# crowsonkb/k-diffusion

Measured on AMD Instinct MI355X. Metric: images/sec, 256x256 image_transformer_v2, 50-step DPM++2M (whole job), higher is better.
Workload: dtype f32

## Files before the change

### k-diffusion_amd/csrc/attn_ffn_x3.hip

```cpp
#include "attn_x3_core.h"
#include "ffn_x3h_core.h"

namespace kd {
namespace x3 {

extern unsigned long long* g_clk;

constexpr int AF_KS = 7;
constexpr int AF_LDS_FFN = 4 * STG + 4 * 1024 + 4 * 2048;
constexpr int AF_LDS = x3a::NaGeo<AF_KS>::LDS > AF_LDS_FFN ? x3a::NaGeo<AF_KS>::LDS : AF_LDS_FFN;
static_assert(AF_LDS <= 80 * 1024, "two workgroups per CU");

struct PanelTile {
  static constexpr bool ATT_LDS = true;
  int tok0, W;
  __device__ __forceinline__ int row(int i) const { return tok0 + (4 * (i >> 6) + ((i & 31) >> 3)) * W + 8 * ((i >> 5) & 1) + (i & 7); }
};

__global__ __launch_bounds__(256, 2) void attn_ffn_x3h_kernel(const x3a::NArgs a, const FArgs3 p) {
  using namespace x3a;
  extern __shared__ __attribute__((aligned(16))) char smem[];
  const int tid = threadIdx.x;
  const auto warm = code_warm_begin<28 * 1024>((int)blockIdx.x < a.warm && tid < 64);
  (void)wg_stamp_begin(a.clk);
  const int tiles_x = a.W / NA_TW, tiles_y = a.H / NA_TH;
  int r = KD_XCD_CHUNK();
  const int tx = r % tiles_x; r /= tiles_x;
  const int ty = r % tiles_y, b = r / tiles_y;
  auto fresh = [&]() { int t = tid; asm volatile("" : "+v"(t)); return t; };

  f32x4 on[2][2][4];
  static_for<2>([&](auto head_) {
    constexpr int head = decltype(head_)::value;
    na2d_x3_tile<AF_KS>(smem, a, fresh(), b, head, ty, tx, [&]() { if constexpr (head == 0) code_warm_end(warm); },
                        [&](bool, int, float l, const f32x16 (&O)[2]) {
      const float inv = 1.0f / l;
#pragma unroll
      for (int e = 0; e < 2; ++e)
#pragma unroll
        for (int g = 0; g < 4; ++g) on[head][e][g] = f32x4(f32x4{O[e][4 * g], O[e][4 * g + 1], O[e][4 * g + 2], O[e][4 * g + 3]} * inv);
    });
    KD_BARRIER();
  });

  const int tid_b = fresh();
  {
    const int lane = tid_b & 63, wid = __builtin_amdgcn_readfirstlane(tid_b >> 6), l31 = lane & 31, h2 = lane >> 5;
    char* rowp = smem + wid * STG + l31 * 512;
#pragma unroll
    for (int head = 0; head < 2; ++head)
#pragma unroll
      for (int e = 0; e < 2; ++e)
#pragma unroll
        for (int g = 0; g < 4; ++g)
          *reinterpret_cast<f32x4*>(rowp + (((16 * head + 8 * e + 2 * g + h2) ^ (l31 & 15)) << 4)) = on[head][e][g];
  }
  asm volatile("s_waitcnt lgkmcnt(0)\n\t; kd_phase_b" ::: "memory");

  ffn_x3h_body<true>(p, smem, tid_b, PanelTile{(b * a.H + ty * NA_TH) * a.W + tx * NA_TW, a.W}, []() {});
  wg_stamp_end(wg_stamp_again(a.clk));
}

}
}

using namespace kd;

extern "C" int kd_attn_ffn_f32_supported(int batch, int H, int W, int nh, int ks, int K, int d_ff) {
  if (!opt(KD_OPT_attn_ffn_x3) || !opt(KD_OPT_attn_x3) || !opt(KD_OPT_ffn_x3)) return 0;
  if (ks != x3::AF_KS || nh != 2 || K != 128 || d_ff <= 0 || (d_ff & 63)) return 0;
  if (batch <= 0 || H <= 0 || W <= 0 || H % x3a::NA_TH || W % x3a::NA_TW) return 0;
  return kd_ffn_f32_supported(batch * H * W, K, d_ff);
}

extern "C" int kd_attn_ffn_f32(const float* qkv, const KdFfn* dp, int batch, int H, int W, int nh, int ks, void* stream) {
  if (!qkv || !dp) return fail(KD_EINVAL, "kd_attn_ffn_f32: null qkv / descriptor");
  const KdFfn& d = *dp;
  if (!d.x || !d.out || !d.scale || !d.Wp_up || !d.Wp_down || !d.Wp_out) return fail(KD_EINVAL, "kd_attn_ffn_f32: null x / out / scale / Wp_up / Wp_down / Wp_out");
  if (ks != x3::AF_KS || nh != 2 || d.K != 128 || d.d_ff <= 0 || (d.d_ff & 63) || batch <= 0 || H <= 0 || W <= 0 || H % x3a::NA_TH || W % x3a::NA_TW)
    return fail(KD_EINVAL, "kd_attn_ffn_f32: kernel size 7, 2 heads of 64, K = 128, d_ff a multiple of 64, token grid a multiple of 8 x 16 (ks=%d nh=%d K=%d d_ff=%d H=%d W=%d)",
                ks, nh, d.K, d.d_ff, H, W);
  if ((long long)batch * H * W != d.M || d.rows_per_sample != H * W || (d.scale_stride & 3))
    return fail(KD_EINVAL, "kd_attn_ffn_f32: M = batch H W, rows_per_sample = H W, scale_stride %% 4 == 0");
  x3a::NArgs a{qkv, nullptr, batch, H, W, nh, code_warm(), x3::g_clk};
  x3::FArgs3 f{};
  f.X = reinterpret_cast<const float*>(d.x); f.Y = reinterpret_cast<float*>(d.out);
  f.Wu = reinterpret_cast<const char*>(d.Wp_up); f.Wd = reinterpret_cast<const char*>(d.Wp_down);
  f.scale = d.scale; f.scale_stride = d.scale_stride; f.rows_per_sample = d.rows_per_sample; f.eps = d.eps;
  f.M = d.M; f.d_ff = d.d_ff; f.n_tiles = d.d_ff / 64;
  f.warm = 0;
  f.clk = x3::g_clk;
  f.Wo = reinterpret_cast<const char*>(d.Wp_out);
  const double M = d.M, K = d.K;
  const double flops = 4.0 * M * nh * x3a::DH * ks * ks + 2.0 * M * 3.0 * d.d_ff * K + 2.0 * M * K * K;
  const double bytes = 16.0 * M * nh * x3a::DH + 4.0 * (3.0 * M * K + 3.0 * d.d_ff * K + K * K) - 8.0 * M * K;
  const ProfName nm("attn_ffn_x3", "attn_ffn_x3 %dx%d nh=%d K=%d d_ff=%d", H, W, nh, d.K, d.d_ff);
  LaunchScope prof(nm, flops, bytes, (hipStream_t)stream);
  launch<x3::attn_ffn_x3h_kernel>(dim3((unsigned)(d.M / 128)), dim3(256), x3::AF_LDS, (hipStream_t)stream, a, f);
  return check_launch("kd_attn_ffn_f32");
}

KD_TEXT_PAD(attn_ffn_x3)
```

### k-diffusion_amd/csrc/attn_x3_core.h

```cpp
#pragma once
#include "x3_common.h"

namespace kd {
namespace x3a {


using b16::bf16x8;
using b16::u32x2;
using b16::u32x4;

constexpr int DH = 64;
constexpr int NA_TH = 8, NA_TW = 16;
constexpr int ROWB = 256;
template <int KS>
struct NaGeo {
  static constexpr int HR = NA_TH + KS - 1, HC = NA_TW + KS - 1;
  static constexpr int PR = 4 + KS - 1;
  static constexpr int NKT = (PR * 16 + 31) / 32;
  static constexpr int ROWS = ((HR * HC - KS + 9 + 3) / 4) * 4;
  static constexpr int LDS = ROWS * ROWB;
  static_assert(8 + KS - 1 <= 16, "16-key patch rows");
};

struct NArgs {
  const float* qkv; float* out;
  int batch, H, W, nh;
  int warm;
  unsigned long long* clk;
};

#define KD_WAIT_VM(n) asm volatile("s_waitcnt vmcnt(" #n ")" ::: "memory")

__device__ __forceinline__ void glds16(const void* src, void* dst) {
  __builtin_amdgcn_global_load_lds((const __attribute__((address_space(1))) void*)src, (__attribute__((address_space(3))) void*)dst, 16, 0, 0);
}

__device__ __forceinline__ int rsw(int row) { return ((row & 3) << 2) | ((row >> 2) & 3); }

using s16x4 = short __attribute__((ext_vector_type(4)));
__device__ __forceinline__ u32x2 tr_read(const char* img, int addr) {
  return __builtin_bit_cast(u32x2, __builtin_amdgcn_ds_read_tr16_b64_v4i16((s16x4 __attribute__((address_space(3)))*)(img + addr)));
}
__device__ __forceinline__ float max3f(float a, float b, float c) { return __builtin_fmaxf(__builtin_fmaxf(a, b), c); }
__device__ __forceinline__ float min3f(float a, float b, float c) { return __builtin_fminf(__builtin_fminf(a, b), c); }


template <int KS, class Mid, class Sink>
__device__ __forceinline__ void na2d_x3_tile(char* img, const NArgs& a, int tid, int b, int head, int ty, int tx, Mid&& mid, Sink&& sink) {
  using G = NaGeo<KS>;
  constexpr int HR = G::HR, HC = G::HC, PR = G::PR, NKT = G::NKT, ROWS = G::ROWS;
  const int lane = tid & 63, wid = __builtin_amdgcn_readfirstlane(tid >> 6), l31 = lane & 31, h2 = lane >> 5;
  const int wy_ = wid >> 1, wx_ = wid & 1;
  const int T = a.H * a.W;
  const size_t row_bytes = (size_t)3 * a.nh * DH * 4;
  const char* base = reinterpret_cast<const char*>(a.qkv) + (size_t)b * T * row_bytes + head * (DH * 4);
  const int ty0 = ty * NA_TH, tx0 = tx * NA_TW;
  const int hy0 = max(0, min(ty0 - KS / 2, a.H - HR)), hx0 = max(0, min(tx0 - KS / 2, a.W - HC));

  constexpr int NPC = (ROWS / 4 + 3) / 4;
  unsigned soff[NPC];
  {
    int row = 4 * wid + (lane >> 4);
    int y = row / HC, x = row % HC;
#pragma unroll
    for (int i = 0; i < NPC; ++i) {
      const int ky = min(hy0 + y, a.H - 1), kx = min(hx0 + x, a.W - 1);
      soff[i] = (unsigned)((ky * a.W + kx) * (int)row_bytes + (((lane & 15) ^ rsw(x)) << 4));
      x += 16;
      if (x >= HC) { x -= HC; ++y; }
    }
  }
  auto stage = [&](int part_bytes) {
#pragma unroll
    for (int i = 0; i < NPC; ++i) {
      const int pc = wid + 4 * i;
      if (pc < ROWS / 4) glds16(base + (size_t)soff[i] + part_bytes, img + pc * 1024);
    }
  };
  stage(a.nh * DH * 4);
  const int qy_raw = ty0 + 4 * wy_ + (l31 >> 3), qx_raw = tx0 + 8 * wx_ + (l31 & 7);
  const bool q_ok = qy_raw < a.H && qx_raw < a.W;
  const int qy = min(qy_raw, a.H - 1), qx = min(qx_raw, a.W - 1);
  const int q_tok = qy * a.W + qx;
  bf16x8 qa[4][2], ql[4];
  {
    const u32x4* qp = reinterpret_cast<const u32x4*>(base + (size_t)q_tok * row_bytes + 32 * h2);
#pragma unroll
    for (int st = 0; st < 4; ++st) {
      const u32x4 c0 = qp[4 * st], c1 = qp[4 * st + 1];
      qa[st][0] = __builtin_bit_cast(bf16x8, u32x4{c0[0], c0[1], c0[0], c0[1]});
      qa[st][1] = __builtin_bit_cast(bf16x8, u32x4{c1[0], c1[1], c1[0], c1[1]});
      ql[st] = __builtin_bit_cast(bf16x8, u32x4{c0[2], c0[3], c1[2], c1[3]});
    }
  }
  const int wy = max(0, min(qy - KS / 2, a.H - KS)) - hy0, wx = max(0, min(qx - KS / 2, a.W - KS)) - hx0;
  const int row_lo = min(max(0, min(min(ty0 + 4 * wy_, a.H - 1) - KS / 2, a.H - KS)) - hy0, HR - PR);
  const int col_lo = min(max(0, min(min(tx0 + 8 * wx_, a.W - 1) - KS / 2, a.W - KS)) - hx0, HC - (8 + KS - 1));
  const int korg = row_lo * HC + col_lo;
  float colv[8], rowv[2 * NKT];
  {
    const int r0 = wy - row_lo, c0 = wx - col_lo;
#pragma unroll
    for (int j = 0; j < 8; ++j) colv[j] = ((unsigned)((j & 3) + 8 * (j >> 2) + 4 * h2 - c0) < (unsigned)KS) ? INFINITY : -INFINITY;
#pragma unroll
    for (int p = 0; p < 2 * NKT; ++p) rowv[p] = ((unsigned)(p - r0) < (unsigned)KS) ? INFINITY : -INFINITY;
  }
  KD_WAIT_VM(0);
  mid();
  KD_BARRIER();

  f32x16 S[NKT];
#pragma unroll
  for (int t = 0; t < NKT; ++t)
#pragma unroll
    for (int i = 0; i < 16; ++i) S[t][i] = 0.f;
  const int kr0 = korg + (l31 >> 4) * HC + (l31 & 15);
  const int ka0 = kr0 * ROWB + (((2 * h2) ^ rsw(col_lo + (l31 & 15))) << 4);
#pragma unroll
  for (int st = 0; st < 4; ++st) {
    bf16x8 kc0[NKT], kc1[NKT], kh[NKT];
    const char* k0p = img + (ka0 ^ (st << 6));
    const char* k1p = img + (ka0 ^ (st << 6) ^ 16);
#pragma unroll
    for (int t = 0; t < NKT; ++t) {
      const u32x4 c0 = *reinterpret_cast<const u32x4*>(k0p + t * (2 * HC * ROWB));
      const u32x4 c1 = *reinterpret_cast<const u32x4*>(k1p + t * (2 * HC * ROWB));
      kc0[t] = __builtin_bit_cast(bf16x8, c0);
      kc1[t] = __builtin_bit_cast(bf16x8, c1);
      kh[t] = __builtin_bit_cast(bf16x8, u32x4{c0[0], c0[1], c1[0], c1[1]});
    }
#pragma unroll
    for (int t = 0; t < NKT; ++t) S[t] = __builtin_amdgcn_mfma_f32_32x32x16_bf16(kc0[t], qa[st][0], S[t], 0, 0, 0);
#pragma unroll
    for (int t = 0; t < NKT; ++t) S[t] = __builtin_amdgcn_mfma_f32_32x32x16_bf16(kc1[t], qa[st][1], S[t], 0, 0, 0);
#pragma unroll
    for (int t = 0; t < NKT; ++t) S[t] = __builtin_amdgcn_mfma_f32_32x32x16_bf16(kh[t], ql[st], S[t], 0, 0, 0);
  }
  asm volatile("s_waitcnt lgkmcnt(0)" ::: "memory");
  KD_BARRIER();
  stage(2 * a.nh * DH * 4);

#pragma unroll
  for (int t = 0; t < NKT; ++t)
#pragma unroll
    for (int i = 0; i < 16; ++i) S[t][i] = min3f(S[t][i], colv[i & 7], rowv[2 * t + (i >> 3)]);
  float m = -INFINITY;
#pragma unroll
  for (int t = 0; t < NKT; ++t)
#pragma unroll
    for (int i = 0; i < 16; i += 2) m = max3f(m, S[t][i], S[t][i + 1]);
  m = fmaxf(m, __shfl_xor(m, 32, 64));
  float l;
  {
    constexpr float LOG2E = 1.4426950408889634f;
    const f32x2 mb = {-m * LOG2E, -m * LOG2E};
    f32x2 l2 = {0.f, 0.f};
#pragma unroll
    for (int t = 0; t < NKT; ++t)
#pragma unroll
      for (int i = 0; i < 16; i += 2) {
        const f32x2 x = __builtin_elementwise_fma(f32x2{S[t][i], S[t][i + 1]}, f32x2{LOG2E, LOG2E}, mb);
        const f32x2 pv = {__builtin_amdgcn_exp2f(x.x), __builtin_amdgcn_exp2f(x.y)};
        S[t][i] = pv.x;
        S[t][i + 1] = pv.y;
        l2 += pv;
      }
    l = l2.x + l2.y;
  }
  l += __shfl_xor(l, 32, 64);
  bf16x8 ph[NKT][2], pl[NKT][2];
#pragma unroll
  for (int t = 0; t < NKT; ++t)
#pragma unroll
    for (int u = 0; u < 2; ++u) {
      u32x4 hi, lo;
      x3::split8(f32x4{S[t][8 * u], S[t][8 * u + 1], S[t][8 * u + 2], S[t][8 * u + 3]},
                 f32x4{S[t][8 * u + 4], S[t][8 * u + 5], S[t][8 * u + 6], S[t][8 * u + 7]}, hi, lo);
      ph[t][u] = __builtin_bit_cast(bf16x8, hi);
      pl[t][u] = __builtin_bit_cast(bf16x8, lo);
    }
  KD_WAIT_VM(0);
  KD_BARRIER();

  f32x16 O[2];
#pragma unroll
  for (int e = 0; e < 2; ++e)
#pragma unroll
    for (int i = 0; i < 16; ++i) O[e][i] = 0.f;
  const int vr0 = korg + 4 * h2 + ((lane & 15) >> 2);
  const int vc = (lane & 3) + 4 * ((lane >> 4) & 1);
  const int va0 = vr0 * ROWB + ((vc ^ rsw(col_lo + 4 * h2 + ((lane & 15) >> 2))) << 4);
  const int vb[2][2] = {{va0, (va0 ^ 32) + 8 * ROWB}, {va0 ^ 128, ((va0 ^ 128) ^ 32) + 8 * ROWB}};
#pragma unroll
  for (int t = 0; t < NKT; ++t)
#pragma unroll
    for (int u = 0; u < 2; ++u) {
      constexpr int step = HC * ROWB;
      bf16x8 vh[2], vl[2];
#pragma unroll
      for (int e = 0; e < 2; ++e) {
        const int a0 = vb[e][0] + (2 * t + u) * step, a1 = vb[e][1] + (2 * t + u) * step;
        const u32x2 h0 = tr_read(img, a0), h1 = tr_read(img, a1), l0 = tr_read(img, a0 + 8), l1 = tr_read(img, a1 + 8);
        vh[e] = __builtin_bit_cast(bf16x8, u32x4{h0[0], h0[1], h1[0], h1[1]});
        vl[e] = __builtin_bit_cast(bf16x8, u32x4{l0[0], l0[1], l1[0], l1[1]});
      }
      O[0] = __builtin_amdgcn_mfma_f32_32x32x16_bf16(vl[0], ph[t][u], O[0], 0, 0, 0);
      O[1] = __builtin_amdgcn_mfma_f32_32x32x16_bf16(vl[1], ph[t][u], O[1], 0, 0, 0);
      O[0] = __builtin_amdgcn_mfma_f32_32x32x16_bf16(vh[0], pl[t][u], O[0], 0, 0, 0);
      O[1] = __builtin_amdgcn_mfma_f32_32x32x16_bf16(vh[1], pl[t][u], O[1], 0, 0, 0);
      O[0] = __builtin_amdgcn_mfma_f32_32x32x16_bf16(vh[0], ph[t][u], O[0], 0, 0, 0);
      O[1] = __builtin_amdgcn_mfma_f32_32x32x16_bf16(vh[1], ph[t][u], O[1], 0, 0, 0);
    }

  sink(q_ok, q_tok, l, O);
}

}
}
```

### k-diffusion_amd/csrc/check_x3_agpr.py

```python
#!/usr/bin/env python3
import os
import re
import subprocess
import sys
import tempfile

HIPCC = os.environ.get("HIPCC", "/opt/rocm/bin/hipcc")


def main(src):
    with tempfile.TemporaryDirectory() as tmp:
        out = os.path.join(tmp, "x3.s")
        subprocess.run([HIPCC, "--offload-arch=" + os.environ.get("ARCH", "gfx950"), "-O3", "-std=c++17", "-fPIC", "-Wno-unused-function", "-S",
                        "--cuda-device-only", src, "-o", out], check=True, capture_output=True)
        txt = open(out).read()
    pos = [(m.start(), m.group(1)) for m in re.finditer(r"\n(_ZN2kd2x3[A-Za-z0-9_]+):", txt)]
    checked = 0
    for (st, name), (en, _) in zip(pos, pos[1:] + [(len(txt), "")]):
        if "gemm_x3_astat_kernelILi32E" not in name and "ffn_x3" not in name and "gemm_x3h_kernel" not in name:
            continue
        body = txt[st:en].split(".end_amdhsa_kernel")[0]
        if not re.search(r"\.vgpr_spill_count:\s*0", txt[st:]) and "vgpr_spill_count" in txt[st:en]:
            raise SystemExit(f"check_x3_agpr: {name}: spills")
        fused = "attn_ffn_x3h" in name
        if fused:
            if "kd_phase_b" not in body:
                raise SystemExit(f"check_x3_agpr: {name}: no kd_phase_b marker")
            m = re.search(r"\.amdhsa_next_free_vgpr\s+(\d+)", txt[st:])
            if not m or int(m.group(1)) > 256:
                raise SystemExit(f"check_x3_agpr: {name}: {m.group(1) if m else '?'} registers per lane: no two workgroups per CU")
        inasm, n_mfma, held = False, 0, not fused
        for line in body.split("\n"):
            t = line.strip()
            held |= "kd_phase_b" in t
            if ";;#ASMSTART" in t:
                inasm = True
            elif ";;#ASMEND" in t:
                inasm = False
            elif not t or t.startswith((";", ".")):
                continue
            elif inasm:
                n_mfma += "v_mfma" in t
            elif "scratch_" in t or (held and (re.search(r"\ba\[?\d", t) or "accvgpr" in t)):
                raise SystemExit(f"check_x3_agpr: {name}: the compiler touches an AccVGPR / scratch outside the kernel's asm: {t}")
        if n_mfma == 0:
            raise SystemExit(f"check_x3_agpr: {name}: no asm MFMA found (did the kernel change?)")
        checked += 1
    if checked == 0:
        raise SystemExit("check_x3_agpr: no named-AccVGPR kernel found in " + src)
    print(f"check_x3_agpr: {os.path.basename(src)}: {checked} named-AccVGPR kernels: a0..a255 are the kernel's alone, no scratch: ok")


if __name__ == "__main__":
    for f in sys.argv[1:]:
        main(f)
```

### k-diffusion_amd/csrc/ffn_x3.hip

```cpp
#include "x3_common.h"
#include "ffn_x3h_core.h"

namespace kd {
namespace x3 {

template <int IDX>
__device__ __forceinline__ void mfma_acc_ag(const bf16x8 w, const bf16x8 h) {
  asm volatile("v_mfma_f32_32x32x16_bf16 a[%c2:%c3], %0, %1, a[%c2:%c3]" :: "v"(w), "v"(h), "i"(IDX), "i"(IDX + 15) : KD_AGPR_ALL);
}
template <int IDX>
__device__ __forceinline__ void areg_zero16() {
  static_for<16>([&](auto i_) { asm volatile("v_accvgpr_write_b32 a[%c0], 0" :: "i"(IDX + decltype(i_)::value) : KD_AGPR_ALL); });
}
template <int IDX, int BIDX>
__device__ __forceinline__ void mfma_acc_aa(const bf16x8 w) {
  asm volatile("v_mfma_f32_32x32x16_bf16 a[%c1:%c2], %0, a[%c3:%c4], a[%c1:%c2]" :: "v"(w), "i"(IDX), "i"(IDX + 15), "i"(BIDX), "i"(BIDX + 3) : KD_AGPR_ALL);
}

template <int NC , bool OUTP = false >
__global__ __launch_bounds__(256, 1) void ffn_x3_kernel(const FArgs3 p) {
  static_assert(!OUTP || NC == 16, "fused out projection: width 256 here, width 128 in ffn_x3h_kernel");
  constexpr int K = NC * 16, NKU = NC / 2;
  constexpr int NOB = K / 32, NKD = 2 * (K / 128);
  constexpr int UNIT = NKU + NKD;
  constexpr int NSTG = 8, PDIST = NSTG - 1, PB = 4;
  constexpr bool AG = NC >= 16;
  constexpr int AO = AG ? 8 * NC : 0;
  constexpr int WAREA = (NSTG / 4) * STG;
  constexpr int KH = WAREA / 128 >= K ? K : WAREA / 128, NR = K / KH, CPR = KH / 4, PIECES = 32 * CPR / 64;
  constexpr int SCL = K * 4 < 1024 ? 1024 : K * 4;
  constexpr int EARLY = K == 128 ? 4 : 0;
  static_assert(NR == 1 && (K == 128 || K == 256), "widths 128 and 256");
  static_assert(UNIT <= 2 * NSTG, "slot arithmetic below assumes at most two trips round the ring per tile");
  extern __shared__ __attribute__((aligned(16))) char smem[];
  const int tid = threadIdx.x, lane = tid & 63, l31 = lane & 31, lh = lane >> 5;
  const int wid = __builtin_amdgcn_readfirstlane(tid >> 6);
  const auto warm = code_warm_begin<(NC <= 8 ? 16 : 28) * 1024>((int)blockIdx.x < p.warm && tid < 64);
  const int m0 = blockIdx.x * 128;
  const int T = p.n_tiles, total = T * UNIT;
  const bool probe = p.clk && blockIdx.x == (gridDim.x * 5) / 8 && tid == 0;
  if (probe) { p.clk[0] = __builtin_amdgcn_s_memtime(); p.clk[1] = __builtin_amdgcn_s_memrealtime(); }
  const WgStamp wgs = wg_stamp_begin(p.clk);

  auto issue_rel = [&](int t, int off, int j) {
    int tt = t + off / UNIT, u = off % UNIT;
    if (tt >= T) { tt = T - 1; u = UNIT - 1; }
    const char* src = (u < NKU ? p.Wu + ((size_t)tt * NKU + u) * STG
                               : p.Wd + ((size_t)((u - NKU) >> 1) * (2 * T) + 2 * tt + ((u - NKU) & 1)) * STG) + wid * (PB * 1024) + lane * 16;
    char* dst = smem + ((t * UNIT + off) % NSTG) * STG + wid * (PB * 1024);
    __builtin_amdgcn_global_load_lds((const __attribute__((address_space(1))) void*)(src + j * 1024),
                                     (__attribute__((address_space(3))) void*)(dst + j * 1024), 16, 0, 0);
  };

  const int row = m0 + wid * 32 + l31;
  const bool ok = row < p.M;
  const int rowc = ok ? row : p.M - 1;
  bf16x8 a_hi[AG ? 1 : NC], a_lo[AG ? 1 : NC];
  float rs = 1.f;
  f32x4 xres[OUTP ? NOB : 1][4];
  if constexpr (OUTP) {
    const float* xr = p.X + (size_t)rowc * K + 4 * lh;
#pragma unroll
    for (int ob = 0; ob < NOB; ++ob)
#pragma unroll
      for (int g = 0; g < 4; ++g) xres[ob][g] = *reinterpret_cast<const f32x4*>(xr + 32 * ob + 8 * g);
  }
  {
    char* stage = smem + (EARLY ? EARLY * STG + wid * STG : wid * WAREA);
    char* scl = smem + NSTG * STG + wid * SCL;
    const int r_first = min(m0 + wid * 32, p.M - 1), r_last = min(m0 + wid * 32 + 31, p.M - 1);
    const bool uni = p.scale_stride == 0 || r_first / p.rows_per_sample == r_last / p.rows_per_sample;
    if (uni) {
      const char* ssrc = reinterpret_cast<const char*>(p.scale + (size_t)(r_first / p.rows_per_sample) * p.scale_stride);
#pragma unroll
      for (int i = 0; i < SCL / 1024; ++i)
        __builtin_amdgcn_global_load_lds((const __attribute__((address_space(1))) void*)(ssrc + (i * 1024 + lane * 16) % (K * 4)),
                                         (__attribute__((address_space(3))) void*)(scl + i * 1024), 16, 0, 0);
    }
    const float* sp = p.scale + (size_t)(rowc / p.rows_per_sample) * p.scale_stride + 8 * lh;
    const float* spl = reinterpret_cast<const float*>(scl) + 8 * lh;
    float ssq = 0.f;
#pragma unroll
    for (int i = 0; i < PIECES; ++i) {
      const int ci = i * 64 + lane, rr = ci / CPR, qs = ci % CPR;
      const int grow = min(m0 + wid * 32 + rr, p.M - 1);
      const char* src = reinterpret_cast<const char*>((OUTP ? p.Att : p.X) + (size_t)grow * K) + ((qs ^ (rr & 15)) << 4);
      __builtin_amdgcn_global_load_lds((const __attribute__((address_space(1))) void*)src,
                                       (__attribute__((address_space(3))) void*)(stage + i * 1024), 16, 0, 0);
    }
    if constexpr (EARLY > 0) {
#pragma unroll
      for (int s = 0; s < EARLY; ++s)
#pragma unroll
        for (int j = 0; j < PB; ++j) issue_rel(0, s, j);
      wait_vm(PB * EARLY);
    } else {
      asm volatile("s_waitcnt vmcnt(0)" ::: "memory");
    }
    const char* rowp = stage + l31 * (KH * 4);
    static_for<NC / 4>([&](auto c4_) {
      constexpr int c0 = 4 * decltype(c4_)::value;
      f32x4 x0[4], x1[4], s0[4], s1[4];
#pragma unroll
      for (int u = 0; u < 4; ++u) {
        const int q = 4 * (c0 + u) + 2 * lh;
        x0[u] = *reinterpret_cast<const f32x4*>(rowp + ((q ^ (l31 & 15)) << 4));
        x1[u] = *reinterpret_cast<const f32x4*>(rowp + (((q + 1) ^ (l31 & 15)) << 4));
        if constexpr (!OUTP) {
          if (uni) {
            s0[u] = *reinterpret_cast<const f32x4*>(spl + 16 * (c0 + u));
            s1[u] = *reinterpret_cast<const f32x4*>(spl + 16 * (c0 + u) + 4);
          } else {
            s0[u] = *reinterpret_cast<const f32x4*>(sp + 16 * (c0 + u));
            s1[u] = *reinterpret_cast<const f32x4*>(sp + 16 * (c0 + u) + 4);
          }
        }
      }
      __builtin_amdgcn_sched_barrier(0);
      static_for<4>([&](auto u_) {
        constexpr int u = decltype(u_)::value;
        u32x4 hi, lo;
        if constexpr (OUTP) {
          split8(x0[u], x1[u], hi, lo);
        } else {
#pragma unroll
          for (int e = 0; e < 4; ++e) ssq = fmaf(x0[u][e], x0[u][e], fmaf(x1[u][e], x1[u][e], ssq));
          split8(x0[u] * s0[u], x1[u] * s1[u], hi, lo);
        }
        if constexpr (AG) {
          areg_write4<8 * (c0 + u)>(hi);
          areg_write4<8 * (c0 + u) + 4>(lo);
        } else {
          asm volatile("" : "+v"(hi), "+v"(lo));
          a_hi[c0 + u] = __builtin_bit_cast(bf16x8, hi);
          a_lo[c0 + u] = __builtin_bit_cast(bf16x8, lo);
        }
      });
      __builtin_amdgcn_sched_barrier(0);
    });
    if constexpr (!OUTP) {
      ssq += __shfl_xor(ssq, 32, 64);
      rs = rsqrtf(ssq / (float)K + p.eps);
    }
  }
  if constexpr (OUTP) {
    static_for<NOB>([&](auto ob_) {
      static_for<4>([&](auto g_) {
        constexpr int ob = decltype(ob_)::value, gq = decltype(g_)::value;
        areg_write4<AO + 16 * ob + 4 * gq>(__builtin_bit_cast(u32x4, xres[ob][gq]));
      });
    });
  } else {
    static_for<NOB>([&](auto ob_) { areg_zero16<AO + 16 * decltype(ob_)::value>(); });
  }
  code_warm_end(warm);
  asm volatile("s_waitcnt vmcnt(0) lgkmcnt(0)" ::: "memory");
  KD_BARRIER();
  constexpr int NWO = OUTP ? 2 * NKU : 0;
  auto issue_wo = [&](int q, int j) {
    const char* src = p.Wo + (size_t)q * STG + wid * (PB * 1024) + j * 1024 + lane * 16;
    char* dst = smem + (q % NSTG) * STG + wid * (PB * 1024) + j * 1024;
    __builtin_amdgcn_global_load_lds((const __attribute__((address_space(1))) void*)src, (__attribute__((address_space(3))) void*)dst, 16, 0, 0);
  };
  if constexpr (OUTP) {
#pragma unroll
    for (int q = 0; q < PDIST; ++q)
#pragma unroll
      for (int j = 0; j < PB; ++j) issue_wo(q, j);
  } else {
#pragma unroll
    for (int s = EARLY; s < PDIST; ++s)
#pragma unroll
      for (int j = 0; j < PB; ++j) issue_rel(0, s, j);
  }
  if (probe) p.clk[4] = __builtin_amdgcn_s_memtime();

  const int o0 = swz64(l31, lh), o1 = swz64(l31, 2 + lh);
  f32x16 acc[4];
  bf16x8 wh[2][4], wl[2][4];
  auto read_frags = [&](int slot, int h, bf16x8 (&fh)[4], bf16x8 (&fl)[4]) {
    const char* st = smem + slot * STG + (h ? o1 : o0);
#pragma unroll
    for (int j = 0; j < 4; ++j) {
      fh[j] = *reinterpret_cast<const bf16x8*>(st + j * 32 * 64);
      fl[j] = *reinterpret_cast<const bf16x8*>(st + IMG + j * 32 * 64);
    }
  };
  auto next_stage_in = [&]() {
    wait_vm(PB * (PDIST - 2));
    KD_BARRIER();
  };
  wait_vm(PB * (PDIST - 1));
  KD_BARRIER();
  read_frags(0, 0, wh[0], wl[0]);
  if constexpr (OUTP) {
    constexpr std::integral_constant<int, 0> I0{};
    constexpr std::integral_constant<int, 1> I1{};
    constexpr std::integral_constant<int, 2> I2{};
    constexpr std::integral_constant<int, 3> I3{};
    static_for<NWO>([&](auto q_) {
      constexpr int q = decltype(q_)::value, ntile = q / NKU, ks = q % NKU;
      auto oo = [&](auto b_, auto j_, bool w_lo, auto al_) {
        constexpr int b = decltype(b_)::value, j = decltype(j_)::value, al = decltype(al_)::value, c = 2 * ks + b;
        mfma_acc_aa<AO + 16 * (4 * ntile + j), 8 * c + 4 * al>(w_lo ? wl[b][j] : wh[b][j]);
      };
      auto request = [&](int j) {
        if constexpr (q + PDIST < NWO) issue_wo(q + PDIST, j);
        else issue_rel(0, q + PDIST - NWO, j);
      };
      oo(I0, I0, true, I0);
      __builtin_amdgcn_sched_barrier(0);
      read_frags(q % NSTG, 1, wh[1], wl[1]);
      __builtin_amdgcn_sched_barrier(0);
      oo(I0, I1, true, I0); oo(I0, I2, true, I0); oo(I0, I3, true, I0);
      oo(I0, I0, false, I1); oo(I0, I1, false, I1); oo(I0, I2, false, I1); oo(I0, I3, false, I1);
      oo(I0, I0, false, I0); oo(I0, I1, false, I0); oo(I0, I2, false, I0); oo(I0, I3, false, I0);
      __builtin_amdgcn_sched_barrier(0);
      next_stage_in();
      oo(I1, I0, true, I0);
      __builtin_amdgcn_sched_barrier(0);
      read_frags((q + 1) % NSTG, 0, wh[0], wl[0]);
      __builtin_amdgcn_sched_barrier(0);
      oo(I1, I1, true, I0); oo(I1, I2, true, I0);
      request(0);
      __builtin_amdgcn_sched_barrier(0);
      oo(I1, I3, true, I0); oo(I1, I0, false, I1); oo(I1, I1, false, I1);
      request(1);
      __builtin_amdgcn_sched_barrier(0);
      oo(I1, I2, false, I1); oo(I1, I3, false, I1); oo(I1, I0, false, I0);
      request(2);
      __builtin_amdgcn_sched_barrier(0);
      oo(I1, I1, false, I0); oo(I1, I2, false, I0);
      request(3);
      oo(I1, I3, false, I0);
      __builtin_amdgcn_sched_barrier(0);
    });
    asm volatile("s_nop 15\n\ts_nop 3" ::: "memory");
    {
      const char* scl = smem + NSTG * STG + wid * SCL;
      const int r_first = min(m0 + wid * 32, p.M - 1), r_last = min(m0 + wid * 32 + 31, p.M - 1);
      const bool uni = p.scale_stride == 0 || r_first / p.rows_per_sample == r_last / p.rows_per_sample;
      const float* sg = uni ? nullptr : p.scale + (size_t)(rowc / p.rows_per_sample) * p.scale_stride + 4 * lh;
      const float* sl = reinterpret_cast<const float*>(scl) + 4 * lh;
      float ssq = 0.f;
      static_for<NOB>([&](auto ob_) {
        constexpr int ob = decltype(ob_)::value;
        f32x4 v[4], sc[4];
        static_for<4>([&](auto g_) { v[decltype(g_)::value] = areg_read4<AO + 16 * ob + 4 * decltype(g_)::value>(); });
#pragma unroll
        for (int g = 0; g < 4; ++g) sc[g] = uni ? *reinterpret_cast<const f32x4*>(sl + 32 * ob + 8 * g) : *reinterpret_cast<const f32x4*>(sg + 32 * ob + 8 * g);
#pragma unroll
        for (int g = 0; g < 4; ++g)
#pragma unroll
          for (int e = 0; e < 4; ++e) ssq = fmaf(v[g][e], v[g][e], ssq);
        static_for<2>([&](auto hc_) {
          constexpr int hc = decltype(hc_)::value;
          u32x4 hi, lo;
          split8(v[2 * hc] * sc[2 * hc], v[2 * hc + 1] * sc[2 * hc + 1], hi, lo);
          areg_write4<8 * (2 * ob + hc)>(hi);
          areg_write4<8 * (2 * ob + hc) + 4>(lo);
        });
      });
      ssq += __shfl_xor(ssq, 32, 64);
      rs = rsqrtf(ssq / (float)K + p.eps);
    }
  }
  const float rsh = 0.5f * rs;

  for (int t = 0; t < T; ++t) {
    const int sbase = t * UNIT;
    const int slot0 = sbase % NSTG;
    if (probe && t == 2) p.clk[8] = __builtin_amdgcn_s_memtime();
    static_for<NKU>([&](auto ks_) {
      constexpr int ks = decltype(ks_)::value;
      const int slot = (slot0 + ks) % NSTG, nslot = (slot0 + ks + 1) % NSTG;
      auto mm = [&](auto b_, int j, bool w_lo, auto a_lo_) {
        constexpr int b = decltype(b_)::value, al = decltype(a_lo_)::value, c = 2 * ks + b;
        const bf16x8& w = w_lo ? wl[b][j] : wh[b][j];
        constexpr bool first = ks == 0 && b == 0;
        if constexpr (AG) {
          if (first && w_lo) mfma_ag0<8 * c + 4 * al>(acc[j], w);
          else mfma_ag<8 * c + 4 * al>(acc[j], w);
        } else {
          if (first && w_lo) mfma_vv0(acc[j], w, al ? a_lo[c] : a_hi[c]);
          else mfma_vv(acc[j], w, al ? a_lo[c] : a_hi[c]);
        }
      };
      constexpr std::integral_constant<int, 0> I0{};
      constexpr std::integral_constant<int, 1> I1{};
      mm(I0, 0, true, I0);
      __builtin_amdgcn_sched_barrier(0);
      read_frags(slot, 1, wh[1], wl[1]);
      __builtin_amdgcn_sched_barrier(0);
#pragma unroll
      for (int j = 1; j < 4; ++j) mm(I0, j, true, I0);
#pragma unroll
      for (int j = 0; j < 4; ++j) mm(I0, j, false, I1);
#pragma unroll
      for (int j = 0; j < 4; ++j) mm(I0, j, false, I0);
      __builtin_amdgcn_sched_barrier(0);
      next_stage_in();
      mm(I1, 0, true, I0);
      __builtin_amdgcn_sched_barrier(0);
      read_frags(nslot, 0, wh[0], wl[0]);
      __builtin_amdgcn_sched_barrier(0);
      mm(I1, 1, true, I0);
      mm(I1, 2, true, I0);
      issue_rel(t, ks + PDIST, 0);
      __builtin_amdgcn_sched_barrier(0);
      mm(I1, 3, true, I0);
      mm(I1, 0, false, I1);
      mm(I1, 1, false, I1);
      issue_rel(t, ks + PDIST, 1);
      __builtin_amdgcn_sched_barrier(0);
      mm(I1, 2, false, I1);
      mm(I1, 3, false, I1);
      mm(I1, 0, false, I0);
      issue_rel(t, ks + PDIST, 2);
      __builtin_amdgcn_sched_barrier(0);
      mm(I1, 1, false, I0);
      mm(I1, 2, false, I0);
      issue_rel(t, ks + PDIST, 3);
      mm(I1, 3, false, I0);
      __builtin_amdgcn_sched_barrier(0);
    });
    asm volatile("s_nop 15\n\ts_nop 3" : "+v"(acc[0]), "+v"(acc[1]), "+v"(acc[2]), "+v"(acc[3]));
    if (probe && t == 0) p.clk[5] = __builtin_amdgcn_s_memtime();
    if (probe && t == 2) p.clk[9] = __builtin_amdgcn_s_memtime();

    bf16x8 hf_hi[4], hf_lo[4];
#pragma unroll
    for (int jj = 0; jj < 2; ++jj)
#pragma unroll
      for (int hc = 0; hc < 2; ++hc) {
        f32x4 v0, v1;
        const int r0 = 8 * hc;
        {
          const f32x2 a = geglu_pair(f32x2{acc[2 * jj][r0], acc[2 * jj][r0 + 1]} * rsh, f32x2{acc[2 * jj + 1][r0], acc[2 * jj + 1][r0 + 1]} * rs);
          const f32x2 b = geglu_pair(f32x2{acc[2 * jj][r0 + 2], acc[2 * jj][r0 + 3]} * rsh, f32x2{acc[2 * jj + 1][r0 + 2], acc[2 * jj + 1][r0 + 3]} * rs);
          v0 = f32x4{a.x, a.y, b.x, b.y};
        }
        {
          const f32x2 a = geglu_pair(f32x2{acc[2 * jj][r0 + 4], acc[2 * jj][r0 + 5]} * rsh, f32x2{acc[2 * jj + 1][r0 + 4], acc[2 * jj + 1][r0 + 5]} * rs);
          const f32x2 b = geglu_pair(f32x2{acc[2 * jj][r0 + 6], acc[2 * jj][r0 + 7]} * rsh, f32x2{acc[2 * jj + 1][r0 + 6], acc[2 * jj + 1][r0 + 7]} * rs);
          v1 = f32x4{a.x, a.y, b.x, b.y};
        }
        u32x4 hi, lo;
        split8(v0, v1, hi, lo);
        hf_hi[2 * jj + hc] = __builtin_bit_cast(bf16x8, hi);
        hf_lo[2 * jj + hc] = __builtin_bit_cast(bf16x8, lo);
      }
    asm volatile("s_nop 7" : "+v"(hf_hi[0]), "+v"(hf_hi[1]), "+v"(hf_hi[2]), "+v"(hf_hi[3]), "+v"(hf_lo[0]), "+v"(hf_lo[1]), "+v"(hf_lo[2]), "+v"(hf_lo[3]));
    __builtin_amdgcn_sched_barrier(0);
    if (probe && t == 2) p.clk[10] = __builtin_amdgcn_s_memtime();

    static_for<NKD>([&](auto v_) {
      constexpr int v = decltype(v_)::value, ntile = v >> 1, kk = v & 1;
      const int slot = (slot0 + NKU + v) % NSTG, nslot = (slot0 + NKU + v + 1) % NSTG;
      auto dd = [&](auto b_, auto j_, bool w_lo, bool h_lo) {
        constexpr int b = decltype(b_)::value, j = decltype(j_)::value;
        const bf16x8& w = w_lo ? wl[b][j] : wh[b][j];
        const bf16x8& h = h_lo ? hf_lo[2 * kk + b] : hf_hi[2 * kk + b];
        mfma_acc_ag<AO + 16 * (4 * ntile + j)>(w, h);
      };
      constexpr std::integral_constant<int, 0> I0{};
      constexpr std::integral_constant<int, 1> I1{};
      constexpr std::integral_constant<int, 2> I2{};
      constexpr std::integral_constant<int, 3> I3{};
      dd(I0, I0, true, false);
      __builtin_amdgcn_sched_barrier(0);
      read_frags(slot, 1, wh[1], wl[1]);
      __builtin_amdgcn_sched_barrier(0);
      dd(I0, I1, true, false); dd(I0, I2, true, false); dd(I0, I3, true, false);
      dd(I0, I0, false, true); dd(I0, I1, false, true); dd(I0, I2, false, true); dd(I0, I3, false, true);
      dd(I0, I0, false, false); dd(I0, I1, false, false); dd(I0, I2, false, false); dd(I0, I3, false, false);
      __builtin_amdgcn_sched_barrier(0);
      next_stage_in();
      dd(I1, I0, true, false);
      __builtin_amdgcn_sched_barrier(0);
      read_frags(nslot, 0, wh[0], wl[0]);
      __builtin_amdgcn_sched_barrier(0);
      dd(I1, I1, true, false); dd(I1, I2, true, false);
      issue_rel(t, NKU + v + PDIST, 0);
      __builtin_amdgcn_sched_barrier(0);
      dd(I1, I3, true, false); dd(I1, I0, false, true); dd(I1, I1, false, true);
      issue_rel(t, NKU + v + PDIST, 1);
      __builtin_amdgcn_sched_barrier(0);
      dd(I1, I2, false, true); dd(I1, I3, false, true); dd(I1, I0, false, false);
      issue_rel(t, NKU + v + PDIST, 2);
      __builtin_amdgcn_sched_barrier(0);
      dd(I1, I1, false, false); dd(I1, I2, false, false);
      issue_rel(t, NKU + v + PDIST, 3);
      dd(I1, I3, false, false);
      __builtin_amdgcn_sched_barrier(0);
    });
    if (probe && t == 0) p.clk[6] = __builtin_amdgcn_s_memtime();
    if (probe && t == 2) p.clk[11] = __builtin_amdgcn_s_memtime();
  }
  if (probe) p.clk[12] = __builtin_amdgcn_s_memtime();
  char* strip = smem + NSTG * STG + 4 * SCL + wid * 2048;
  float* st_row[2];
  const float* sk_row[2];
  bool st_ok[2];
#pragma unroll
  for (int it = 0; it < 2; ++it) {
    const int r = m0 + wid * 32 + 16 * it + (lane >> 2);
    st_ok[it] = r < p.M;
    st_row[it] = p.Y + (size_t)min(r, p.M - 1) * K + 4 * (lane & 3);
    sk_row[it] = p.X + (size_t)min(r, p.M - 1) * K + 4 * (lane & 3);
  }
  f32x4 skip_all[NOB][2][2];
#pragma unroll
  for (int ob = 0; ob < NOB; ++ob)
#pragma unroll
    for (int hb = 0; hb < 2; ++hb)
#pragma unroll
      for (int it = 0; it < 2; ++it)
        skip_all[ob][hb][it] = OUTP ? f32x4{0.f, 0.f, 0.f, 0.f} : *reinterpret_cast<const f32x4*>(sk_row[it] + 32 * ob + 16 * hb);
  __builtin_amdgcn_sched_barrier(0);
  asm volatile("s_waitcnt vmcnt(0)\n\ts_nop 15\n\ts_nop 3" ::: "memory");
  static_for<NOB>([&](auto ob_) {
    constexpr int ob = decltype(ob_)::value;
    f32x4 blk[4];
    static_for<4>([&](auto g_) { blk[decltype(g_)::value] = areg_read4<AO + 16 * ob + 4 * decltype(g_)::value>(); });
#pragma unroll
    for (int hb = 0; hb < 2; ++hb) {
      const f32x4 (&skip)[2] = skip_all[ob][hb];
#pragma unroll
      for (int gg = 0; gg < 2; ++gg)
        *reinterpret_cast<f32x4*>(strip + l31 * 64 + (((2 * gg + lh) ^ ((l31 >> 2) & 1)) << 4)) = blk[2 * hb + gg];
#pragma unroll
      for (int it = 0; it < 2; ++it) {
        const int r16 = 16 * it + (lane >> 2), c = lane & 3;
        const f32x4 o = *reinterpret_cast<const f32x4*>(strip + r16 * 64 + ((c ^ ((r16 >> 2) & 1)) << 4));
        if (st_ok[it]) st16(st_row[it] + 32 * ob + 16 * hb, f32x4(o + skip[it]));
      }
    }
  });
  if (probe) { p.clk[2] = __builtin_amdgcn_s_memtime(); p.clk[3] = __builtin_amdgcn_s_memrealtime(); p.clk[7] = (unsigned long long)total; }
  wg_stamp_end(wgs);
}


template <bool OUTP>
__global__ __launch_bounds__(256, 2) void ffn_x3h_kernel(const FArgs3 p) {
  extern __shared__ __attribute__((aligned(16))) char smem[];
  const auto warm = code_warm_begin<16 * 1024>((int)blockIdx.x < p.warm && threadIdx.x < 64);
  const WgStamp wgs = wg_stamp_begin(p.clk);
  ffn_x3h_body<OUTP>(p, smem, (int)threadIdx.x, PanelRows{(int)blockIdx.x * 128}, [&]() { code_warm_end(warm); });
  wg_stamp_end(wgs);
}

extern unsigned long long* g_clk;

template <bool OUTP>
static int launch_ffn_half(const FArgs3& a, const char* nm, double flops, double bytes, hipStream_t s) {
  constexpr int LDS = 4 * STG + 4 * 1024 + 4 * 2048;
  const CfgName cfg(nm, "half1");
  LaunchScope prof(cfg, flops, bytes, s);
  launch<ffn_x3h_kernel<OUTP>>(dim3((unsigned)((a.M + 127) / 128)), dim3(256), LDS, s, a);
  return check_launch("kd_ffn_f32");
}

template <int NC, bool OUTP = false>
static int launch_ffn(const FArgs3& a, const char* nm, double flops, double bytes, hipStream_t s) {
  constexpr int K = NC * 16;
  constexpr int LDS = 8 * STG + 4 * (K * 4 < 1024 ? 1024 : K * 4) + 4 * 2048;
  const CfgName cfg(nm, "half0");
  LaunchScope prof(cfg, flops, bytes, s);
  launch<ffn_x3_kernel<NC, OUTP>>(dim3((unsigned)((a.M + 127) / 128)), dim3(256), LDS, s, a);
  return check_launch("kd_ffn_f32");
}

}
}

using namespace kd;

extern "C" int kd_ffn_f32_supported(int M, int K, int d_ff) {
  if (!opt(KD_OPT_ffn_x3)) return 0;
  if (!((K == 128 || K == 256) && d_ff > 0 && d_ff % 64 == 0)) return 0;
  if (K == 128) return M >= 2048;
  int dev = 0, cus = 256;
  (void)hipGetDevice(&dev);
  if (hipDeviceGetAttribute(&cus, hipDeviceAttributeMultiprocessorCount, dev) != hipSuccess || cus <= 0) cus = 256;
  const int need = opt_or(KD_OPT_ffn_x3_min_panels_256, cus - cus / 8);
  return (M + 127) / 128 >= need;
}

extern "C" int kd_ffn_f32(const KdFfn* dp, void* stream) {
  if (!dp) return fail(KD_EINVAL, "kd_ffn_f32: null descriptor");
  const KdFfn& d = *dp;
  if (!d.x || !d.out || !d.scale || !d.Wp_up || !d.Wp_down) return fail(KD_EINVAL, "kd_ffn_f32: null x / out / scale / Wp_up / Wp_down");
  if ((d.K != 128 && d.K != 256) || d.d_ff <= 0 || (d.d_ff & 63) || d.M <= 0) return fail(KD_EINVAL, "kd_ffn_f32: K must be 128 or 256, d_ff a multiple of 64 (K=%d d_ff=%d)", d.K, d.d_ff);
  if (d.rows_per_sample <= 0 || (d.scale_stride & 3)) return fail(KD_EINVAL, "kd_ffn_f32: rows_per_sample > 0, scale_stride %% 4 == 0");
  x3::FArgs3 a{};
  a.X = reinterpret_cast<const float*>(d.x); a.Y = reinterpret_cast<float*>(d.out);
  a.Wu = reinterpret_cast<const char*>(d.Wp_up); a.Wd = reinterpret_cast<const char*>(d.Wp_down);
  a.scale = d.scale; a.scale_stride = d.scale_stride; a.rows_per_sample = d.rows_per_sample; a.eps = d.eps;
  a.M = d.M; a.d_ff = d.d_ff; a.n_tiles = d.d_ff / 64;
  a.warm = code_warm();
  a.clk = x3::g_clk;
  const double flops = 2.0 * d.M * 3.0 * d.d_ff * d.K;
  const double bytes = 4.0 * (2.0 * d.M * d.K + 3.0 * d.d_ff * d.K);
  const ProfName nm("ffn_x3", "%s M=%d K=%d d_ff=%d", d.attn ? "ffn_x3+out" : "ffn_x3", d.M, d.K, d.d_ff);
  if (d.attn) {
    if (!d.Wp_out) return fail(KD_EINVAL, "kd_ffn_f32: attn without Wp_out");
    a.Att = reinterpret_cast<const float*>(d.attn); a.Wo = reinterpret_cast<const char*>(d.Wp_out);
    const double fl2 = flops + 2.0 * d.M * d.K * d.K, by2 = 4.0 * (3.0 * d.M * d.K + 3.0 * d.d_ff * d.K + (double)d.K * d.K);
    if (d.K == 128) return x3::launch_ffn_half<true>(a, nm, fl2, by2, (hipStream_t)stream);
    return x3::launch_ffn<16, true>(a, nm, fl2, by2, (hipStream_t)stream);
  }
  if (d.K == 128 && opt(KD_OPT_ffn_x3_half)) return x3::launch_ffn_half<false>(a, nm, flops, bytes, (hipStream_t)stream);
  if (d.K == 128) return x3::launch_ffn<8>(a, nm, flops, bytes, (hipStream_t)stream);
  return x3::launch_ffn<16>(a, nm, flops, bytes, (hipStream_t)stream);
}

KD_TEXT_PAD(ffn_x3)
```

Measured before the change: 237.7.

## Fuse neighborhood attention with FFN at width 256 and pipeline heads

Adds a fused attention+FFN kernel for 4 heads at K=256. It runs the four neighborhood-attention heads back to back and then the FFN with output projection in the same workgroup, avoiding a round trip of the attention output through global memory and a separate launch. The attention tile gains an optional pipelined mode that double-buffers V in LDS and prefetches the next head's Q and K while the current head finishes. The FFN body is moved into a shared header so both kernels can use it. The new kernel uses more LDS and registers and runs one workgroup per CU, which lowers occupancy.

```diff
diff --git a/k-diffusion_amd/csrc/attn_ffn_x3.hip b/k-diffusion_amd/csrc/attn_ffn_x3.hip
--- a/k-diffusion_amd/csrc/attn_ffn_x3.hip
+++ b/k-diffusion_amd/csrc/attn_ffn_x3.hip
@@ -1,5 +1,6 @@
 #include "attn_x3_core.h"
 #include "ffn_x3h_core.h"
+#include "ffn_x3_core.h"
 
 namespace kd {
 namespace x3 {
@@ -7,6 +8,7 @@
 extern unsigned long long* g_clk;
 
 constexpr int AF_KS = 7;
+constexpr bool af_width(int nh, int K) { return (nh == 2 && K == 128) || (nh == 4 && K == 256); }
 constexpr int AF_LDS_FFN = 4 * STG + 4 * 1024 + 4 * 2048;
 constexpr int AF_LDS = x3a::NaGeo<AF_KS>::LDS > AF_LDS_FFN ? x3a::NaGeo<AF_KS>::LDS : AF_LDS_FFN;
 static_assert(AF_LDS <= 80 * 1024, "two workgroups per CU");
@@ -61,6 +63,55 @@
   wg_stamp_end(wg_stamp_again(a.clk));
 }
 
+constexpr int AF256_LDS_FFN = 8 * STG + 4 * 1024 + 4 * 2048, AF256_LDS_A = 2 * x3a::NaGeo<AF_KS>::LDS;
+constexpr int AF256_LDS = AF256_LDS_A > AF256_LDS_FFN ? AF256_LDS_A : AF256_LDS_FFN;
+static_assert(AF256_LDS <= 160 * 1024, "one workgroup per CU");
+
+__global__ __launch_bounds__(256, 1) void attn_ffn_x3_kernel(const x3a::NArgs a, const FArgs3 p) {
+  using namespace x3a;
+  extern __shared__ __attribute__((aligned(16))) char smem[];
+  const int tid = threadIdx.x;
+  const auto warm = code_warm_begin<28 * 1024>((int)blockIdx.x < a.warm && tid < 64);
+  (void)wg_stamp_begin(a.clk);
+  const int tiles_x = a.W / NA_TW, tiles_y = a.H / NA_TH;
+  int r = KD_XCD_CHUNK();
+  const int tx = r % tiles_x; r /= tiles_x;
+  const int ty = r % tiles_y, b = r / tiles_y;
+  auto fresh = [&]() { int t = tid; asm volatile("" : "+v"(t)); return t; };
+
+  f32x4 on[4][2][4];
+  bf16x8 qa[4][2], ql[4];
+  static_for<4>([&](auto head_) {
+    constexpr int head = decltype(head_)::value;
+    na2d_x3_tile<AF_KS>(smem, a, fresh(), b, head, ty, tx, [&]() { if constexpr (head == 0) code_warm_end(warm); },
+                        [&](bool, int, float l, const f32x16 (&O)[2]) {
+      const float inv = 1.0f / l;
+#pragma unroll
+      for (int e = 0; e < 2; ++e)
+#pragma unroll
+        for (int g = 0; g < 4; ++g) on[head][e][g] = f32x4(f32x4{O[e][4 * g], O[e][4 * g + 1], O[e][4 * g + 2], O[e][4 * g + 3]} * inv);
+    }, NaPipe<head == 0, head == 3>{qa, ql});
+    if constexpr (head == 3) KD_BARRIER();
+  });
+
+  const int tid_b = fresh();
+  {
+    const int lane = tid_b & 63, wid = __builtin_amdgcn_readfirstlane(tid_b >> 6), l31 = lane & 31, h2 = lane >> 5;
+    char* rowp = smem + wid * (2 * STG) + l31 * 1024;
+#pragma unroll
+    for (int head = 0; head < 4; ++head)
+#pragma unroll
+      for (int e = 0; e < 2; ++e)
+#pragma unroll
+        for (int g = 0; g < 4; ++g)
+          *reinterpret_cast<f32x4*>(rowp + (((16 * head + 8 * e + 2 * g + h2) ^ (l31 & 15)) << 4)) = on[head][e][g];
+  }
+  asm volatile("s_waitcnt lgkmcnt(0)\n\t; kd_phase_b" ::: "memory");
+
+  ffn_x3_body<16, true>(p, smem, tid_b, PanelTile{(b * a.H + ty * NA_TH) * a.W + tx * NA_TW, a.W}, []() {});
+  wg_stamp_end(wg_stamp_again(a.clk));
+}
+
 }
 }
 
@@ -68,7 +119,7 @@
 
 extern "C" int kd_attn_ffn_f32_supported(int batch, int H, int W, int nh, int ks, int K, int d_ff) {
   if (!opt(KD_OPT_attn_ffn_x3) || !opt(KD_OPT_attn_x3) || !opt(KD_OPT_ffn_x3)) return 0;
-  if (ks != x3::AF_KS || nh != 2 || K != 128 || d_ff <= 0 || (d_ff & 63)) return 0;
+  if (ks != x3::AF_KS || !x3::af_width(nh, K) || d_ff <= 0 || (d_ff & 63)) return 0;
   if (batch <= 0 || H <= 0 || W <= 0 || H % x3a::NA_TH || W % x3a::NA_TW) return 0;
   return kd_ffn_f32_supported(batch * H * W, K, d_ff);
 }
@@ -77,8 +128,8 @@
   if (!qkv || !dp) return fail(KD_EINVAL, "kd_attn_ffn_f32: null qkv / descriptor");
   const KdFfn& d = *dp;
   if (!d.x || !d.out || !d.scale || !d.Wp_up || !d.Wp_down || !d.Wp_out) return fail(KD_EINVAL, "kd_attn_ffn_f32: null x / out / scale / Wp_up / Wp_down / Wp_out");
-  if (ks != x3::AF_KS || nh != 2 || d.K != 128 || d.d_ff <= 0 || (d.d_ff & 63) || batch <= 0 || H <= 0 || W <= 0 || H % x3a::NA_TH || W % x3a::NA_TW)
-    return fail(KD_EINVAL, "kd_attn_ffn_f32: kernel size 7, 2 heads of 64, K = 128, d_ff a multiple of 64, token grid a multiple of 8 x 16 (ks=%d nh=%d K=%d d_ff=%d H=%d W=%d)",
+  if (ks != x3::AF_KS || !x3::af_width(nh, d.K) || d.d_ff <= 0 || (d.d_ff & 63) || batch <= 0 || H <= 0 || W <= 0 || H % x3a::NA_TH || W % x3a::NA_TW)
+    return fail(KD_EINVAL, "kd_attn_ffn_f32: kernel size 7, 2 heads of 64 at K = 128 or 4 at K = 256, d_ff a multiple of 64, token grid a multiple of 8 x 16 (ks=%d nh=%d K=%d d_ff=%d H=%d W=%d)",
                 ks, nh, d.K, d.d_ff, H, W);
   if ((long long)batch * H * W != d.M || d.rows_per_sample != H * W || (d.scale_stride & 3))
     return fail(KD_EINVAL, "kd_attn_ffn_f32: M = batch H W, rows_per_sample = H W, scale_stride %% 4 == 0");
@@ -96,7 +147,8 @@
   const double bytes = 16.0 * M * nh * x3a::DH + 4.0 * (3.0 * M * K + 3.0 * d.d_ff * K + K * K) - 8.0 * M * K;
   const ProfName nm("attn_ffn_x3", "attn_ffn_x3 %dx%d nh=%d K=%d d_ff=%d", H, W, nh, d.K, d.d_ff);
   LaunchScope prof(nm, flops, bytes, (hipStream_t)stream);
-  launch<x3::attn_ffn_x3h_kernel>(dim3((unsigned)(d.M / 128)), dim3(256), x3::AF_LDS, (hipStream_t)stream, a, f);
+  if (d.K == 256) launch<x3::attn_ffn_x3_kernel>(dim3((unsigned)(d.M / 128)), dim3(256), x3::AF256_LDS, (hipStream_t)stream, a, f);
+  else launch<x3::attn_ffn_x3h_kernel>(dim3((unsigned)(d.M / 128)), dim3(256), x3::AF_LDS, (hipStream_t)stream, a, f);
   return check_launch("kd_attn_ffn_f32");
 }
 
diff --git a/k-diffusion_amd/csrc/attn_x3_core.h b/k-diffusion_amd/csrc/attn_x3_core.h
--- a/k-diffusion_amd/csrc/attn_x3_core.h
+++ b/k-diffusion_amd/csrc/attn_x3_core.h
@@ -45,10 +45,21 @@
 __device__ __forceinline__ float min3f(float a, float b, float c) { return __builtin_fminf(__builtin_fminf(a, b), c); }
 
 
-template <int KS, class Mid, class Sink>
-__device__ __forceinline__ void na2d_x3_tile(char* img, const NArgs& a, int tid, int b, int head, int ty, int tx, Mid&& mid, Sink&& sink) {
+struct NaSerial { static constexpr bool PIPE = false, FIRST = true, LAST = true; };
+template <bool FIRST_, bool LAST_>
+struct NaPipe {
+  static constexpr bool PIPE = true, FIRST = FIRST_, LAST = LAST_;
+  bf16x8 (&qa)[4][2];
+  bf16x8 (&ql)[4];
+};
+
+template <int KS, class Mid, class Sink, class Pipe = NaSerial>
+__device__ __forceinline__ void na2d_x3_tile(char* img, const NArgs& a, int tid, int b, int head, int ty, int tx, Mid&& mid, Sink&& sink, Pipe&& pipe = NaSerial{}) {
   using G = NaGeo<KS>;
+  using PP = std::remove_reference_t<Pipe>;
   constexpr int HR = G::HR, HC = G::HC, PR = G::PR, NKT = G::NKT, ROWS = G::ROWS;
+  constexpr int MINP = (ROWS / 4) / 4;
+  char* const img_v = img + (PP::PIPE ? G::LDS : 0);
   const int lane = tid & 63, wid = __builtin_amdgcn_readfirstlane(tid >> 6), l31 = lane & 31, h2 = lane >> 5;
   const int wy_ = wid >> 1, wx_ = wid & 1;
   const int T = a.H * a.W;
@@ -70,21 +81,23 @@
       if (x >= HC) { x -= HC; ++y; }
     }
   }
-  auto stage = [&](int part_bytes) {
+  auto stage = [&](int part_bytes, char* dst) {
 #pragma unroll
     for (int i = 0; i < NPC; ++i) {
       const int pc = wid + 4 * i;
-      if (pc < ROWS / 4) glds16(base + (size_t)soff[i] + part_bytes, img + pc * 1024);
+      if (pc < ROWS / 4) glds16(base + (size_t)soff[i] + part_bytes, dst + pc * 1024);
     }
   };
-  stage(a.nh * DH * 4);
+  if constexpr (!PP::PIPE) stage(a.nh * DH * 4, img);
   const int qy_raw = ty0 + 4 * wy_ + (l31 >> 3), qx_raw = tx0 + 8 * wx_ + (l31 & 7);
   const bool q_ok = qy_raw < a.H && qx_raw < a.W;
   const int qy = min(qy_raw, a.H - 1), qx = min(qx_raw, a.W - 1);
   const int q_tok = qy * a.W + qx;
-  bf16x8 qa[4][2], ql[4];
-  {
-    const u32x4* qp = reinterpret_cast<const u32x4*>(base + (size_t)q_tok * row_bytes + 32 * h2);
+  bf16x8 qa_own[4][2], ql_own[4];
+  auto& qa = [&]() -> bf16x8 (&)[4][2] { if constexpr (PP::PIPE) return pipe.qa; else return qa_own; }();
+  auto& ql = [&]() -> bf16x8 (&)[4] { if constexpr (PP::PIPE) return pipe.ql; else return ql_own; }();
+  auto load_q = [&](int head_off) {
+    const u32x4* qp = reinterpret_cast<const u32x4*>(base + (size_t)q_tok * row_bytes + 32 * h2 + head_off * (DH * 4));
 #pragma unroll
     for (int st = 0; st < 4; ++st) {
       const u32x4 c0 = qp[4 * st], c1 = qp[4 * st + 1];
@@ -92,6 +105,18 @@
       qa[st][1] = __builtin_bit_cast(bf16x8, u32x4{c1[0], c1[1], c1[0], c1[1]});
       ql[st] = __builtin_bit_cast(bf16x8, u32x4{c0[2], c0[3], c1[2], c1[3]});
     }
+  };
+  auto q_arrived = [&]() {
+#pragma unroll
+    for (int st = 0; st < 4; ++st) asm volatile("" : "+v"(qa[st][0]), "+v"(qa[st][1]), "+v"(ql[st]));
+  };
+  if constexpr (!PP::PIPE) {
+    load_q(0);
+  } else if constexpr (PP::FIRST) {
+    load_q(0);
+    stage(a.nh * DH * 4, img);
+    q_arrived();
+    stage(2 * a.nh * DH * 4, img_v);
   }
   const int wy = max(0, min(qy - KS / 2, a.H - KS)) - hy0, wx = max(0, min(qx - KS / 2, a.W - KS)) - hx0;
   const int row_lo = min(max(0, min(min(ty0 + 4 * wy_, a.H - 1) - KS / 2, a.H - KS)) - hy0, HR - PR);
@@ -105,7 +130,8 @@
 #pragma unroll
     for (int p = 0; p < 2 * NKT; ++p) rowv[p] = ((unsigned)(p - r0) < (unsigned)KS) ? INFINITY : -INFINITY;
   }
-  KD_WAIT_VM(0);
+  if constexpr (PP::PIPE) x3::wait_vm(MINP);
+  else KD_WAIT_VM(0);
   mid();
   KD_BARRIER();
 
@@ -138,7 +164,12 @@
   }
   asm volatile("s_waitcnt lgkmcnt(0)" ::: "memory");
   KD_BARRIER();
-  stage(2 * a.nh * DH * 4);
+  if constexpr (!PP::PIPE) {
+    stage(2 * a.nh * DH * 4, img);
+  } else if constexpr (!PP::LAST) {
+    load_q(1);
+    stage(a.nh * DH * 4 + DH * 4, img);
+  }
 
 #pragma unroll
   for (int t = 0; t < NKT; ++t)
@@ -179,7 +210,8 @@
       ph[t][u] = __builtin_bit_cast(bf16x8, hi);
       pl[t][u] = __builtin_bit_cast(bf16x8, lo);
     }
-  KD_WAIT_VM(0);
+  if constexpr (PP::PIPE && !PP::LAST) x3::wait_vm(MINP);
+  else KD_WAIT_VM(0);
   KD_BARRIER();
 
   f32x16 O[2];
@@ -200,7 +232,7 @@
 #pragma unroll
       for (int e = 0; e < 2; ++e) {
         const int a0 = vb[e][0] + (2 * t + u) * step, a1 = vb[e][1] + (2 * t + u) * step;
-        const u32x2 h0 = tr_read(img, a0), h1 = tr_read(img, a1), l0 = tr_read(img, a0 + 8), l1 = tr_read(img, a1 + 8);
+        const u32x2 h0 = tr_read(img_v, a0), h1 = tr_read(img_v, a1), l0 = tr_read(img_v, a0 + 8), l1 = tr_read(img_v, a1 + 8);
         vh[e] = __builtin_bit_cast(bf16x8, u32x4{h0[0], h0[1], h1[0], h1[1]});
         vl[e] = __builtin_bit_cast(bf16x8, u32x4{l0[0], l0[1], l1[0], l1[1]});
       }
@@ -213,7 +245,12 @@
     }
 
   sink(q_ok, q_tok, l, O);
-}
-
-}
-}
+  if constexpr (PP::PIPE && !PP::LAST) {
+    KD_BARRIER();
+    q_arrived();
+    stage(2 * a.nh * DH * 4 + DH * 4, img_v);
+  }
+}
+
+}
+}
diff --git a/k-diffusion_amd/csrc/check_x3_agpr.py b/k-diffusion_amd/csrc/check_x3_agpr.py
--- a/k-diffusion_amd/csrc/check_x3_agpr.py
+++ b/k-diffusion_amd/csrc/check_x3_agpr.py
@@ -22,12 +22,12 @@
         body = txt[st:en].split(".end_amdhsa_kernel")[0]
         if not re.search(r"\.vgpr_spill_count:\s*0", txt[st:]) and "vgpr_spill_count" in txt[st:en]:
             raise SystemExit(f"check_x3_agpr: {name}: spills")
-        fused = "attn_ffn_x3h" in name
+        fused = "attn_ffn_x3" in name
         if fused:
             if "kd_phase_b" not in body:
                 raise SystemExit(f"check_x3_agpr: {name}: no kd_phase_b marker")
             m = re.search(r"\.amdhsa_next_free_vgpr\s+(\d+)", txt[st:])
-            if not m or int(m.group(1)) > 256:
+            if "attn_ffn_x3h" in name and (not m or int(m.group(1)) > 256):
                 raise SystemExit(f"check_x3_agpr: {name}: {m.group(1) if m else '?'} registers per lane: no two workgroups per CU")
         inasm, n_mfma, held = False, 0, not fused
         for line in body.split("\n"):
diff --git a/k-diffusion_amd/csrc/ffn_x3.hip b/k-diffusion_amd/csrc/ffn_x3.hip
--- a/k-diffusion_amd/csrc/ffn_x3.hip
+++ b/k-diffusion_amd/csrc/ffn_x3.hip
@@ -1,446 +1,18 @@
 #include "x3_common.h"
 #include "ffn_x3h_core.h"
+#include "ffn_x3_core.h"
 
 namespace kd {
 namespace x3 {
 
-template <int IDX>
-__device__ __forceinline__ void mfma_acc_ag(const bf16x8 w, const bf16x8 h) {
-  asm volatile("v_mfma_f32_32x32x16_bf16 a[%c2:%c3], %0, %1, a[%c2:%c3]" :: "v"(w), "v"(h), "i"(IDX), "i"(IDX + 15) : KD_AGPR_ALL);
-}
-template <int IDX>
-__device__ __forceinline__ void areg_zero16() {
-  static_for<16>([&](auto i_) { asm volatile("v_accvgpr_write_b32 a[%c0], 0" :: "i"(IDX + decltype(i_)::value) : KD_AGPR_ALL); });
-}
-template <int IDX, int BIDX>
-__device__ __forceinline__ void mfma_acc_aa(const bf16x8 w) {
-  asm volatile("v_mfma_f32_32x32x16_bf16 a[%c1:%c2], %0, a[%c3:%c4], a[%c1:%c2]" :: "v"(w), "i"(IDX), "i"(IDX + 15), "i"(BIDX), "i"(BIDX + 3) : KD_AGPR_ALL);
-}
-
 template <int NC , bool OUTP = false >
 __global__ __launch_bounds__(256, 1) void ffn_x3_kernel(const FArgs3 p) {
-  static_assert(!OUTP || NC == 16, "fused out projection: width 256 here, width 128 in ffn_x3h_kernel");
-  constexpr int K = NC * 16, NKU = NC / 2;
-  constexpr int NOB = K / 32, NKD = 2 * (K / 128);
-  constexpr int UNIT = NKU + NKD;
-  constexpr int NSTG = 8, PDIST = NSTG - 1, PB = 4;
-  constexpr bool AG = NC >= 16;
-  constexpr int AO = AG ? 8 * NC : 0;
-  constexpr int WAREA = (NSTG / 4) * STG;
-  constexpr int KH = WAREA / 128 >= K ? K : WAREA / 128, NR = K / KH, CPR = KH / 4, PIECES = 32 * CPR / 64;
-  constexpr int SCL = K * 4 < 1024 ? 1024 : K * 4;
-  constexpr int EARLY = K == 128 ? 4 : 0;
-  static_assert(NR == 1 && (K == 128 || K == 256), "widths 128 and 256");
-  static_assert(UNIT <= 2 * NSTG, "slot arithmetic below assumes at most two trips round the ring per tile");
   extern __shared__ __attribute__((aligned(16))) char smem[];
-  const int tid = threadIdx.x, lane = tid & 63, l31 = lane & 31, lh = lane >> 5;
-  const int wid = __builtin_amdgcn_readfirstlane(tid >> 6);
-  const auto warm = code_warm_begin<(NC <= 8 ? 16 : 28) * 1024>((int)blockIdx.x < p.warm && tid < 64);
-  const int m0 = blockIdx.x * 128;
-  const int T = p.n_tiles, total = T * UNIT;
-  const bool probe = p.clk && blockIdx.x == (gridDim.x * 5) / 8 && tid == 0;
-  if (probe) { p.clk[0] = __builtin_amdgcn_s_memtime(); p.clk[1] = __builtin_amdgcn_s_memrealtime(); }
+  const auto warm = code_warm_begin<(NC <= 8 ? 16 : 28) * 1024>((int)blockIdx.x < p.warm && threadIdx.x < 64);
   const WgStamp wgs = wg_stamp_begin(p.clk);
-
-  auto issue_rel = [&](int t, int off, int j) {
-    int tt = t + off / UNIT, u = off % UNIT;
-    if (tt >= T) { tt = T - 1; u = UNIT - 1; }
-    const char* src = (u < NKU ? p.Wu + ((size_t)tt * NKU + u) * STG
-                               : p.Wd + ((size_t)((u - NKU) >> 1) * (2 * T) + 2 * tt + ((u - NKU) & 1)) * STG) + wid * (PB * 1024) + lane * 16;
-    char* dst = smem + ((t * UNIT + off) % NSTG) * STG + wid * (PB * 1024);
-    __builtin_amdgcn_global_load_lds((const __attribute__((address_space(1))) void*)(src + j * 1024),
-                                     (__attribute__((address_space(3))) void*)(dst + j * 1024), 16, 0, 0);
-  };
-
-  const int row = m0 + wid * 32 + l31;
-  const bool ok = row < p.M;
-  const int rowc = ok ? row : p.M - 1;
-  bf16x8 a_hi[AG ? 1 : NC], a_lo[AG ? 1 : NC];
-  float rs = 1.f;
-  f32x4 xres[OUTP ? NOB : 1][4];
-  if constexpr (OUTP) {
-    const float* xr = p.X + (size_t)rowc * K + 4 * lh;
-#pragma unroll
-    for (int ob = 0; ob < NOB; ++ob)
-#pragma unroll
-      for (int g = 0; g < 4; ++g) xres[ob][g] = *reinterpret_cast<const f32x4*>(xr + 32 * ob + 8 * g);
-  }
-  {
-    char* stage = smem + (EARLY ? EARLY * STG + wid * STG : wid * WAREA);
-    char* scl = smem + NSTG * STG + wid * SCL;
-    const int r_first = min(m0 + wid * 32, p.M - 1), r_last = min(m0 + wid * 32 + 31, p.M - 1);
-    const bool uni = p.scale_stride == 0 || r_first / p.rows_per_sample == r_last / p.rows_per_sample;
-    if (uni) {
-      const char* ssrc = reinterpret_cast<const char*>(p.scale + (size_t)(r_first / p.rows_per_sample) * p.scale_stride);
-#pragma unroll
-      for (int i = 0; i < SCL / 1024; ++i)
-        __builtin_amdgcn_global_load_lds((const __attribute__((address_space(1))) void*)(ssrc + (i * 1024 + lane * 16) % (K * 4)),
-                                         (__attribute__((address_space(3))) void*)(scl + i * 1024), 16, 0, 0);
-    }
-    const float* sp = p.scale + (size_t)(rowc / p.rows_per_sample) * p.scale_stride + 8 * lh;
-    const float* spl = reinterpret_cast<const float*>(scl) + 8 * lh;
-    float ssq = 0.f;
-#pragma unroll
-    for (int i = 0; i < PIECES; ++i) {
-      const int ci = i * 64 + lane, rr = ci / CPR, qs = ci % CPR;
-      const int grow = min(m0 + wid * 32 + rr, p.M - 1);
-      const char* src = reinterpret_cast<const char*>((OUTP ? p.Att : p.X) + (size_t)grow * K) + ((qs ^ (rr & 15)) << 4);
-      __builtin_amdgcn_global_load_lds((const __attribute__((address_space(1))) void*)src,
-                                       (__attribute__((address_space(3))) void*)(stage + i * 1024), 16, 0, 0);
-    }
-    if constexpr (EARLY > 0) {
-#pragma unroll
-      for (int s = 0; s < EARLY; ++s)
-#pragma unroll
-        for (int j = 0; j < PB; ++j) issue_rel(0, s, j);
-      wait_vm(PB * EARLY);
-    } else {
-      asm volatile("s_waitcnt vmcnt(0)" ::: "memory");
-    }
-    const char* rowp = stage + l31 * (KH * 4);
-    static_for<NC / 4>([&](auto c4_) {
-      constexpr int c0 = 4 * decltype(c4_)::value;
-      f32x4 x0[4], x1[4], s0[4], s1[4];
-#pragma unroll
-      for (int u = 0; u < 4; ++u) {
-        const int q = 4 * (c0 + u) + 2 * lh;
-        x0[u] = *reinterpret_cast<const f32x4*>(rowp + ((q ^ (l31 & 15)) << 4));
-        x1[u] = *reinterpret_cast<const f32x4*>(rowp + (((q + 1) ^ (l31 & 15)) << 4));
-        if constexpr (!OUTP) {
-          if (uni) {
-            s0[u] = *reinterpret_cast<const f32x4*>(spl + 16 * (c0 + u));
-            s1[u] = *reinterpret_cast<const f32x4*>(spl + 16 * (c0 + u) + 4);
-          } else {
-            s0[u] = *reinterpret_cast<const f32x4*>(sp + 16 * (c0 + u));
-            s1[u] = *reinterpret_cast<const f32x4*>(sp + 16 * (c0 + u) + 4);
-          }
-        }
-      }
-      __builtin_amdgcn_sched_barrier(0);
-      static_for<4>([&](auto u_) {
-        constexpr int u = decltype(u_)::value;
-        u32x4 hi, lo;
-        if constexpr (OUTP) {
-          split8(x0[u], x1[u], hi, lo);
-        } else {
-#pragma unroll
-          for (int e = 0; e < 4; ++e) ssq = fmaf(x0[u][e], x0[u][e], fmaf(x1[u][e], x1[u][e], ssq));
-          split8(x0[u] * s0[u], x1[u] * s1[u], hi, lo);
-        }
-        if constexpr (AG) {
-          areg_write4<8 * (c0 + u)>(hi);
-          areg_write4<8 * (c0 + u) + 4>(lo);
-        } else {
-          asm volatile("" : "+v"(hi), "+v"(lo));
-          a_hi[c0 + u] = __builtin_bit_cast(bf16x8, hi);
-          a_lo[c0 + u] = __builtin_bit_cast(bf16x8, lo);
-        }
-      });
-      __builtin_amdgcn_sched_barrier(0);
-    });
-    if constexpr (!OUTP) {
-      ssq += __shfl_xor(ssq, 32, 64);
-      rs = rsqrtf(ssq / (float)K + p.eps);
-    }
-  }
-  if constexpr (OUTP) {
-    static_for<NOB>([&](auto ob_) {
-      static_for<4>([&](auto g_) {
-        constexpr int ob = decltype(ob_)::value, gq = decltype(g_)::value;
-        areg_write4<AO + 16 * ob + 4 * gq>(__builtin_bit_cast(u32x4, xres[ob][gq]));
-      });
-    });
-  } else {
-    static_for<NOB>([&](auto ob_) { areg_zero16<AO + 16 * decltype(ob_)::value>(); });
-  }
-  code_warm_end(warm);
-  asm volatile("s_waitcnt vmcnt(0) lgkmcnt(0)" ::: "memory");
-  KD_BARRIER();
-  constexpr int NWO = OUTP ? 2 * NKU : 0;
-  auto issue_wo = [&](int q, int j) {
-    const char* src = p.Wo + (size_t)q * STG + wid * (PB * 1024) + j * 1024 + lane * 16;
-    char* dst = smem + (q % NSTG) * STG + wid * (PB * 1024) + j * 1024;
-    __builtin_amdgcn_global_load_lds((const __attribute__((address_space(1))) void*)src, (__attribute__((address_space(3))) void*)dst, 16, 0, 0);
-  };
-  if constexpr (OUTP) {
-#pragma unroll
-    for (int q = 0; q < PDIST; ++q)
-#pragma unroll
-      for (int j = 0; j < PB; ++j) issue_wo(q, j);
-  } else {
-#pragma unroll
-    for (int s = EARLY; s < PDIST; ++s)
-#pragma unroll
-      for (int j = 0; j < PB; ++j) issue_rel(0, s, j);
-  }
-  if (probe) p.clk[4] = __builtin_amdgcn_s_memtime();
-
-  const int o0 = swz64(l31, lh), o1 = swz64(l31, 2 + lh);
-  f32x16 acc[4];
-  bf16x8 wh[2][4], wl[2][4];
-  auto read_frags = [&](int slot, int h, bf16x8 (&fh)[4], bf16x8 (&fl)[4]) {
-    const char* st = smem + slot * STG + (h ? o1 : o0);
-#pragma unroll
-    for (int j = 0; j < 4; ++j) {
-      fh[j] = *reinterpret_cast<const bf16x8*>(st + j * 32 * 64);
-      fl[j] = *reinterpret_cast<const bf16x8*>(st + IMG + j * 32 * 64);
-    }
-  };
-  auto next_stage_in = [&]() {
-    wait_vm(PB * (PDIST - 2));
-    KD_BARRIER();
-  };
-  wait_vm(PB * (PDIST - 1));
-  KD_BARRIER();
-  read_frags(0, 0, wh[0], wl[0]);
-  if constexpr (OUTP) {
-    constexpr std::integral_constant<int, 0> I0{};
-    constexpr std::integral_constant<int, 1> I1{};
-    constexpr std::integral_constant<int, 2> I2{};
-    constexpr std::integral_constant<int, 3> I3{};
-    static_for<NWO>([&](auto q_) {
-      constexpr int q = decltype(q_)::value, ntile = q / NKU, ks = q % NKU;
-      auto oo = [&](auto b_, auto j_, bool w_lo, auto al_) {
-        constexpr int b = decltype(b_)::value, j = decltype(j_)::value, al = decltype(al_)::value, c = 2 * ks + b;
-        mfma_acc_aa<AO + 16 * (4 * ntile + j), 8 * c + 4 * al>(w_lo ? wl[b][j] : wh[b][j]);
-      };
-      auto request = [&](int j) {
-        if constexpr (q + PDIST < NWO) issue_wo(q + PDIST, j);
-        else issue_rel(0, q + PDIST - NWO, j);
-      };
-      oo(I0, I0, true, I0);
-      __builtin_amdgcn_sched_barrier(0);
-      read_frags(q % NSTG, 1, wh[1], wl[1]);
-      __builtin_amdgcn_sched_barrier(0);
-      oo(I0, I1, true, I0); oo(I0, I2, true, I0); oo(I0, I3, true, I0);
-      oo(I0, I0, false, I1); oo(I0, I1, false, I1); oo(I0, I2, false, I1); oo(I0, I3, false, I1);
-      oo(I0, I0, false, I0); oo(I0, I1, false, I0); oo(I0, I2, false, I0); oo(I0, I3, false, I0);
-      __builtin_amdgcn_sched_barrier(0);
-      next_stage_in();
-      oo(I1, I0, true, I0);
-      __builtin_amdgcn_sched_barrier(0);
-      read_frags((q + 1) % NSTG, 0, wh[0], wl[0]);
-      __builtin_amdgcn_sched_barrier(0);
-      oo(I1, I1, true, I0); oo(I1, I2, true, I0);
-      request(0);
-      __builtin_amdgcn_sched_barrier(0);
-      oo(I1, I3, true, I0); oo(I1, I0, false, I1); oo(I1, I1, false, I1);
-      request(1);
-      __builtin_amdgcn_sched_barrier(0);
-      oo(I1, I2, false, I1); oo(I1, I3, false, I1); oo(I1, I0, false, I0);
-      request(2);
-      __builtin_amdgcn_sched_barrier(0);
-      oo(I1, I1, false, I0); oo(I1, I2, false, I0);
-      request(3);
-      oo(I1, I3, false, I0);
-      __builtin_amdgcn_sched_barrier(0);
-    });
-    asm volatile("s_nop 15\n\ts_nop 3" ::: "memory");
-    {
-      const char* scl = smem + NSTG * STG + wid * SCL;
-      const int r_first = min(m0 + wid * 32, p.M - 1), r_last = min(m0 + wid * 32 + 31, p.M - 1);
-      const bool uni = p.scale_stride == 0 || r_first / p.rows_per_sample == r_last / p.rows_per_sample;
-      const float* sg = uni ? nullptr : p.scale + (size_t)(rowc / p.rows_per_sample) * p.scale_stride + 4 * lh;
-      const float* sl = reinterpret_cast<const float*>(scl) + 4 * lh;
-      float ssq = 0.f;
-      static_for<NOB>([&](auto ob_) {
-        constexpr int ob = decltype(ob_)::value;
-        f32x4 v[4], sc[4];
-        static_for<4>([&](auto g_) { v[decltype(g_)::value] = areg_read4<AO + 16 * ob + 4 * decltype(g_)::value>(); });
-#pragma unroll
-        for (int g = 0; g < 4; ++g) sc[g] = uni ? *reinterpret_cast<const f32x4*>(sl + 32 * ob + 8 * g) : *reinterpret_cast<const f32x4*>(sg + 32 * ob + 8 * g);
-#pragma unroll
-        for (int g = 0; g < 4; ++g)
-#pragma unroll
-          for (int e = 0; e < 4; ++e) ssq = fmaf(v[g][e], v[g][e], ssq);
-        static_for<2>([&](auto hc_) {
-          constexpr int hc = decltype(hc_)::value;
-          u32x4 hi, lo;
-          split8(v[2 * hc] * sc[2 * hc], v[2 * hc + 1] * sc[2 * hc + 1], hi, lo);
-          areg_write4<8 * (2 * ob + hc)>(hi);
-          areg_write4<8 * (2 * ob + hc) + 4>(lo);
-        });
-      });
-      ssq += __shfl_xor(ssq, 32, 64);
-      rs = rsqrtf(ssq / (float)K + p.eps);
-    }
-  }
-  const float rsh = 0.5f * rs;
-
-  for (int t = 0; t < T; ++t) {
-    const int sbase = t * UNIT;
-    const int slot0 = sbase % NSTG;
-    if (probe && t == 2) p.clk[8] = __builtin_amdgcn_s_memtime();
-    static_for<NKU>([&](auto ks_) {
-      constexpr int ks = decltype(ks_)::value;
-      const int slot = (slot0 + ks) % NSTG, nslot = (slot0 + ks + 1) % NSTG;
-      auto mm = [&](auto b_, int j, bool w_lo, auto a_lo_) {
-        constexpr int b = decltype(b_)::value, al = decltype(a_lo_)::value, c = 2 * ks + b;
-        const bf16x8& w = w_lo ? wl[b][j] : wh[b][j];
-        constexpr bool first = ks == 0 && b == 0;
-        if constexpr (AG) {
-          if (first && w_lo) mfma_ag0<8 * c + 4 * al>(acc[j], w);
-          else mfma_ag<8 * c + 4 * al>(acc[j], w);
-        } else {
-          if (first && w_lo) mfma_vv0(acc[j], w, al ? a_lo[c] : a_hi[c]);
-          else mfma_vv(acc[j], w, al ? a_lo[c] : a_hi[c]);
-        }
-      };
-      constexpr std::integral_constant<int, 0> I0{};
-      constexpr std::integral_constant<int, 1> I1{};
-      mm(I0, 0, true, I0);
-      __builtin_amdgcn_sched_barrier(0);
-      read_frags(slot, 1, wh[1], wl[1]);
-      __builtin_amdgcn_sched_barrier(0);
-#pragma unroll
-      for (int j = 1; j < 4; ++j) mm(I0, j, true, I0);
-#pragma unroll
-      for (int j = 0; j < 4; ++j) mm(I0, j, false, I1);
-#pragma unroll
-      for (int j = 0; j < 4; ++j) mm(I0, j, false, I0);
-      __builtin_amdgcn_sched_barrier(0);
-      next_stage_in();
-      mm(I1, 0, true, I0);
-      __builtin_amdgcn_sched_barrier(0);
-      read_frags(nslot, 0, wh[0], wl[0]);
-      __builtin_amdgcn_sched_barrier(0);
-      mm(I1, 1, true, I0);
-      mm(I1, 2, true, I0);
-      issue_rel(t, ks + PDIST, 0);
-      __builtin_amdgcn_sched_barrier(0);
-      mm(I1, 3, true, I0);
-      mm(I1, 0, false, I1);
-      mm(I1, 1, false, I1);
-      issue_rel(t, ks + PDIST, 1);
-      __builtin_amdgcn_sched_barrier(0);
-      mm(I1, 2, false, I1);
-      mm(I1, 3, false, I1);
-      mm(I1, 0, false, I0);
-      issue_rel(t, ks + PDIST, 2);
-      __builtin_amdgcn_sched_barrier(0);
-      mm(I1, 1, false, I0);
-      mm(I1, 2, false, I0);
-      issue_rel(t, ks + PDIST, 3);
-      mm(I1, 3, false, I0);
-      __builtin_amdgcn_sched_barrier(0);
-    });
-    asm volatile("s_nop 15\n\ts_nop 3" : "+v"(acc[0]), "+v"(acc[1]), "+v"(acc[2]), "+v"(acc[3]));
-    if (probe && t == 0) p.clk[5] = __builtin_amdgcn_s_memtime();
-    if (probe && t == 2) p.clk[9] = __builtin_amdgcn_s_memtime();
-
-    bf16x8 hf_hi[4], hf_lo[4];
-#pragma unroll
-    for (int jj = 0; jj < 2; ++jj)
-#pragma unroll
-      for (int hc = 0; hc < 2; ++hc) {
-        f32x4 v0, v1;
-        const int r0 = 8 * hc;
-        {
-          const f32x2 a = geglu_pair(f32x2{acc[2 * jj][r0], acc[2 * jj][r0 + 1]} * rsh, f32x2{acc[2 * jj + 1][r0], acc[2 * jj + 1][r0 + 1]} * rs);
-          const f32x2 b = geglu_pair(f32x2{acc[2 * jj][r0 + 2], acc[2 * jj][r0 + 3]} * rsh, f32x2{acc[2 * jj + 1][r0 + 2], acc[2 * jj + 1][r0 + 3]} * rs);
-          v0 = f32x4{a.x, a.y, b.x, b.y};
-        }
-        {
-          const f32x2 a = geglu_pair(f32x2{acc[2 * jj][r0 + 4], acc[2 * jj][r0 + 5]} * rsh, f32x2{acc[2 * jj + 1][r0 + 4], acc[2 * jj + 1][r0 + 5]} * rs);
-          const f32x2 b = geglu_pair(f32x2{acc[2 * jj][r0 + 6], acc[2 * jj][r0 + 7]} * rsh, f32x2{acc[2 * jj + 1][r0 + 6], acc[2 * jj + 1][r0 + 7]} * rs);
-          v1 = f32x4{a.x, a.y, b.x, b.y};
-        }
-        u32x4 hi, lo;
-        split8(v0, v1, hi, lo);
-        hf_hi[2 * jj + hc] = __builtin_bit_cast(bf16x8, hi);
-        hf_lo[2 * jj + hc] = __builtin_bit_cast(bf16x8, lo);
-      }
-    asm volatile("s_nop 7" : "+v"(hf_hi[0]), "+v"(hf_hi[1]), "+v"(hf_hi[2]), "+v"(hf_hi[3]), "+v"(hf_lo[0]), "+v"(hf_lo[1]), "+v"(hf_lo[2]), "+v"(hf_lo[3]));
-    __builtin_amdgcn_sched_barrier(0);
-    if (probe && t == 2) p.clk[10] = __builtin_amdgcn_s_memtime();
-
-    static_for<NKD>([&](auto v_) {
-      constexpr int v = decltype(v_)::value, ntile = v >> 1, kk = v & 1;
-      const int slot = (slot0 + NKU + v) % NSTG, nslot = (slot0 + NKU + v + 1) % NSTG;
-      auto dd = [&](auto b_, auto j_, bool w_lo, bool h_lo) {
-        constexpr int b = decltype(b_)::value, j = decltype(j_)::value;
-        const bf16x8& w = w_lo ? wl[b][j] : wh[b][j];
-        const bf16x8& h = h_lo ? hf_lo[2 * kk + b] : hf_hi[2 * kk + b];
-        mfma_acc_ag<AO + 16 * (4 * ntile + j)>(w, h);
-      };
-      constexpr std::integral_constant<int, 0> I0{};
-      constexpr std::integral_constant<int, 1> I1{};
-      constexpr std::integral_constant<int, 2> I2{};
-      constexpr std::integral_constant<int, 3> I3{};
-      dd(I0, I0, true, false);
-      __builtin_amdgcn_sched_barrier(0);
-      read_frags(slot, 1, wh[1], wl[1]);
-      __builtin_amdgcn_sched_barrier(0);
-      dd(I0, I1, true, false); dd(I0, I2, true, false); dd(I0, I3, true, false);
-      dd(I0, I0, false, true); dd(I0, I1, false, true); dd(I0, I2, false, true); dd(I0, I3, false, true);
-      dd(I0, I0, false, false); dd(I0, I1, false, false); dd(I0, I2, false, false); dd(I0, I3, false, false);
-      __builtin_amdgcn_sched_barrier(0);
-      next_stage_in();
-      dd(I1, I0, true, false);
-      __builtin_amdgcn_sched_barrier(0);
-      read_frags(nslot, 0, wh[0], wl[0]);
-      __builtin_amdgcn_sched_barrier(0);
-      dd(I1, I1, true, false); dd(I1, I2, true, false);
-      issue_rel(t, NKU + v + PDIST, 0);
-      __builtin_amdgcn_sched_barrier(0);
-      dd(I1, I3, true, false); dd(I1, I0, false, true); dd(I1, I1, false, true);
-      issue_rel(t, NKU + v + PDIST, 1);
-      __builtin_amdgcn_sched_barrier(0);
-      dd(I1, I2, false, true); dd(I1, I3, false, true); dd(I1, I0, false, false);
-      issue_rel(t, NKU + v + PDIST, 2);
-      __builtin_amdgcn_sched_barrier(0);
-      dd(I1, I1, false, false); dd(I1, I2, false, false);
-      issue_rel(t, NKU + v + PDIST, 3);
-      dd(I1, I3, false, false);
-      __builtin_amdgcn_sched_barrier(0);
-    });
-    if (probe && t == 0) p.clk[6] = __builtin_amdgcn_s_memtime();
-    if (probe && t == 2) p.clk[11] = __builtin_amdgcn_s_memtime();
-  }
-  if (probe) p.clk[12] = __builtin_amdgcn_s_memtime();
-  char* strip = smem + NSTG * STG + 4 * SCL + wid * 2048;
-  float* st_row[2];
-  const float* sk_row[2];
-  bool st_ok[2];
-#pragma unroll
-  for (int it = 0; it < 2; ++it) {
-    const int r = m0 + wid * 32 + 16 * it + (lane >> 2);
-    st_ok[it] = r < p.M;
-    st_row[it] = p.Y + (size_t)min(r, p.M - 1) * K + 4 * (lane & 3);
-    sk_row[it] = p.X + (size_t)min(r, p.M - 1) * K + 4 * (lane & 3);
-  }
-  f32x4 skip_all[NOB][2][2];
-#pragma unroll
-  for (int ob = 0; ob < NOB; ++ob)
-#pragma unroll
-    for (int hb = 0; hb < 2; ++hb)
-#pragma unroll
-      for (int it = 0; it < 2; ++it)
-        skip_all[ob][hb][it] = OUTP ? f32x4{0.f, 0.f, 0.f, 0.f} : *reinterpret_cast<const f32x4*>(sk_row[it] + 32 * ob + 16 * hb);
-  __builtin_amdgcn_sched_barrier(0);
-  asm volatile("s_waitcnt vmcnt(0)\n\ts_nop 15\n\ts_nop 3" ::: "memory");
-  static_for<NOB>([&](auto ob_) {
-    constexpr int ob = decltype(ob_)::value;
-    f32x4 blk[4];
-    static_for<4>([&](auto g_) { blk[decltype(g_)::value] = areg_read4<AO + 16 * ob + 4 * decltype(g_)::value>(); });
-#pragma unroll
-    for (int hb = 0; hb < 2; ++hb) {
-      const f32x4 (&skip)[2] = skip_all[ob][hb];
-#pragma unroll
-      for (int gg = 0; gg < 2; ++gg)
-        *reinterpret_cast<f32x4*>(strip + l31 * 64 + (((2 * gg + lh) ^ ((l31 >> 2) & 1)) << 4)) = blk[2 * hb + gg];
-#pragma unroll
-      for (int it = 0; it < 2; ++it) {
-        const int r16 = 16 * it + (lane >> 2), c = lane & 3;
-        const f32x4 o = *reinterpret_cast<const f32x4*>(strip + r16 * 64 + ((c ^ ((r16 >> 2) & 1)) << 4));
-        if (st_ok[it]) st16(st_row[it] + 32 * ob + 16 * hb, f32x4(o + skip[it]));
-      }
-    }
-  });
-  if (probe) { p.clk[2] = __builtin_amdgcn_s_memtime(); p.clk[3] = __builtin_amdgcn_s_memrealtime(); p.clk[7] = (unsigned long long)total; }
+  ffn_x3_body<NC, OUTP>(p, smem, (int)threadIdx.x, PanelRows{(int)blockIdx.x * 128}, [&]() { code_warm_end(warm); });
   wg_stamp_end(wgs);
 }
-
 
 template <bool OUTP>
 __global__ __launch_bounds__(256, 2) void ffn_x3h_kernel(const FArgs3 p) {
diff --git a/k-diffusion_amd/csrc/ffn_x3_core.h b/k-diffusion_amd/csrc/ffn_x3_core.h
--- /dev/null
+++ b/k-diffusion_amd/csrc/ffn_x3_core.h
@@ -0,0 +1,444 @@
+#pragma once
+#include "x3_common.h"
+#include "ffn_x3h_core.h"
+
+namespace kd {
+namespace x3 {
+
+template <int IDX>
+__device__ __forceinline__ void mfma_acc_ag(const bf16x8 w, const bf16x8 h) {
+  asm volatile("v_mfma_f32_32x32x16_bf16 a[%c2:%c3], %0, %1, a[%c2:%c3]" :: "v"(w), "v"(h), "i"(IDX), "i"(IDX + 15) : KD_AGPR_ALL);
+}
+template <int IDX>
+__device__ __forceinline__ void areg_zero16() {
+  static_for<16>([&](auto i_) { asm volatile("v_accvgpr_write_b32 a[%c0], 0" :: "i"(IDX + decltype(i_)::value) : KD_AGPR_ALL); });
+}
+template <int IDX, int BIDX>
+__device__ __forceinline__ void mfma_acc_aa(const bf16x8 w) {
+  asm volatile("v_mfma_f32_32x32x16_bf16 a[%c1:%c2], %0, a[%c3:%c4], a[%c1:%c2]" :: "v"(w), "i"(IDX), "i"(IDX + 15), "i"(BIDX), "i"(BIDX + 3) : KD_AGPR_ALL);
+}
+
+template <int NC , bool OUTP , class Panel, class WarmEnd>
+__device__ __forceinline__ void ffn_x3_body(const FArgs3& p, char* smem, int tid, const Panel& pn, WarmEnd&& warm_end) {
+  static_assert(!OUTP || NC == 16, "fused out projection: width 256 here, width 128 in ffn_x3h_kernel");
+  static_assert(!Panel::ATT_LDS || OUTP, "attention rows in LDS: the fused out projection's operand");
+  constexpr int K = NC * 16, NKU = NC / 2;
+  constexpr int NOB = K / 32, NKD = 2 * (K / 128);
+  constexpr int UNIT = NKU + NKD;
+  constexpr int NSTG = 8, PDIST = NSTG - 1, PB = 4;
+  constexpr bool AG = NC >= 16;
+  constexpr int AO = AG ? 8 * NC : 0;
+  constexpr int WAREA = (NSTG / 4) * STG;
+  constexpr int KH = WAREA / 128 >= K ? K : WAREA / 128, NR = K / KH, CPR = KH / 4, PIECES = 32 * CPR / 64;
+  constexpr int SCL = K * 4 < 1024 ? 1024 : K * 4;
+  constexpr int EARLY = K == 128 ? 4 : 0;
+  static_assert(NR == 1 && (K == 128 || K == 256), "widths 128 and 256");
+  static_assert(UNIT <= 2 * NSTG, "slot arithmetic below assumes at most two trips round the ring per tile");
+  const int lane = tid & 63, l31 = lane & 31, lh = lane >> 5;
+  const int wid = __builtin_amdgcn_readfirstlane(tid >> 6);
+  const int T = p.n_tiles, total = T * UNIT;
+  const bool probe = p.clk && blockIdx.x == (gridDim.x * 5) / 8 && tid == 0;
+  if (probe) { p.clk[0] = __builtin_amdgcn_s_memtime(); p.clk[1] = __builtin_amdgcn_s_memrealtime(); }
+
+  auto issue_rel = [&](int t, int off, int j) {
+    int tt = t + off / UNIT, u = off % UNIT;
+    if (tt >= T) { tt = T - 1; u = UNIT - 1; }
+    const char* src = (u < NKU ? p.Wu + ((size_t)tt * NKU + u) * STG
+                               : p.Wd + ((size_t)((u - NKU) >> 1) * (2 * T) + 2 * tt + ((u - NKU) & 1)) * STG) + wid * (PB * 1024) + lane * 16;
+    char* dst = smem + ((t * UNIT + off) % NSTG) * STG + wid * (PB * 1024);
+    __builtin_amdgcn_global_load_lds((const __attribute__((address_space(1))) void*)(src + j * 1024),
+                                     (__attribute__((address_space(3))) void*)(dst + j * 1024), 16, 0, 0);
+  };
+
+  const int row = pn.row(wid * 32 + l31);
+  const bool ok = row < p.M;
+  const int rowc = ok ? row : p.M - 1;
+  bf16x8 a_hi[AG ? 1 : NC], a_lo[AG ? 1 : NC];
+  float rs = 1.f;
+  f32x4 xres[OUTP ? NOB : 1][4];
+  if constexpr (OUTP) {
+    const float* xr = p.X + (size_t)rowc * K + 4 * lh;
+#pragma unroll
+    for (int ob = 0; ob < NOB; ++ob)
+#pragma unroll
+      for (int g = 0; g < 4; ++g) xres[ob][g] = *reinterpret_cast<const f32x4*>(xr + 32 * ob + 8 * g);
+  }
+  {
+    char* stage = smem + (EARLY ? EARLY * STG + wid * STG : wid * WAREA);
+    char* scl = smem + NSTG * STG + wid * SCL;
+    const int r_first = min(pn.row(wid * 32), p.M - 1), r_last = min(pn.row(wid * 32 + 31), p.M - 1);
+    const bool uni = p.scale_stride == 0 || r_first / p.rows_per_sample == r_last / p.rows_per_sample;
+    if (uni) {
+      const char* ssrc = reinterpret_cast<const char*>(p.scale + (size_t)(r_first / p.rows_per_sample) * p.scale_stride);
+#pragma unroll
+      for (int i = 0; i < SCL / 1024; ++i)
+        __builtin_amdgcn_global_load_lds((const __attribute__((address_space(1))) void*)(ssrc + (i * 1024 + lane * 16) % (K * 4)),
+                                         (__attribute__((address_space(3))) void*)(scl + i * 1024), 16, 0, 0);
+    }
+    const float* sp = p.scale + (size_t)(rowc / p.rows_per_sample) * p.scale_stride + 8 * lh;
+    const float* spl = reinterpret_cast<const float*>(scl) + 8 * lh;
+    float ssq = 0.f;
+    if constexpr (!Panel::ATT_LDS) {
+#pragma unroll
+      for (int i = 0; i < PIECES; ++i) {
+        const int ci = i * 64 + lane, rr = ci / CPR, qs = ci % CPR;
+        const int grow = min(pn.row(wid * 32 + rr), p.M - 1);
+        const char* src = reinterpret_cast<const char*>((OUTP ? p.Att : p.X) + (size_t)grow * K) + ((qs ^ (rr & 15)) << 4);
+        __builtin_amdgcn_global_load_lds((const __attribute__((address_space(1))) void*)src,
+                                         (__attribute__((address_space(3))) void*)(stage + i * 1024), 16, 0, 0);
+      }
+    }
+    if constexpr (EARLY > 0) {
+#pragma unroll
+      for (int s = 0; s < EARLY; ++s)
+#pragma unroll
+        for (int j = 0; j < PB; ++j) issue_rel(0, s, j);
+      wait_vm(PB * EARLY);
+    } else {
+      asm volatile("s_waitcnt vmcnt(0)" ::: "memory");
+    }
+    const char* rowp = stage + l31 * (KH * 4);
+    static_for<NC / 4>([&](auto c4_) {
+      constexpr int c0 = 4 * decltype(c4_)::value;
+      f32x4 x0[4], x1[4], s0[4], s1[4];
+#pragma unroll
+      for (int u = 0; u < 4; ++u) {
+        const int q = 4 * (c0 + u) + 2 * lh;
+        x0[u] = *reinterpret_cast<const f32x4*>(rowp + ((q ^ (l31 & 15)) << 4));
+        x1[u] = *reinterpret_cast<const f32x4*>(rowp + (((q + 1) ^ (l31 & 15)) << 4));
+        if constexpr (!OUTP) {
+          if (uni) {
+            s0[u] = *reinterpret_cast<const f32x4*>(spl + 16 * (c0 + u));
+            s1[u] = *reinterpret_cast<const f32x4*>(spl + 16 * (c0 + u) + 4);
+          } else {
+            s0[u] = *reinterpret_cast<const f32x4*>(sp + 16 * (c0 + u));
+            s1[u] = *reinterpret_cast<const f32x4*>(sp + 16 * (c0 + u) + 4);
+          }
+        }
+      }
+      __builtin_amdgcn_sched_barrier(0);
+      static_for<4>([&](auto u_) {
+        constexpr int u = decltype(u_)::value;
+        u32x4 hi, lo;
+        if constexpr (OUTP) {
+          split8(x0[u], x1[u], hi, lo);
+        } else {
+#pragma unroll
+          for (int e = 0; e < 4; ++e) ssq = fmaf(x0[u][e], x0[u][e], fmaf(x1[u][e], x1[u][e], ssq));
+          split8(x0[u] * s0[u], x1[u] * s1[u], hi, lo);
+        }
+        if constexpr (AG) {
+          areg_write4<8 * (c0 + u)>(hi);
+          areg_write4<8 * (c0 + u) + 4>(lo);
+        } else {
+          asm volatile("" : "+v"(hi), "+v"(lo));
+          a_hi[c0 + u] = __builtin_bit_cast(bf16x8, hi);
+          a_lo[c0 + u] = __builtin_bit_cast(bf16x8, lo);
+        }
+      });
+      __builtin_amdgcn_sched_barrier(0);
+    });
+    if constexpr (!OUTP) {
+      ssq += __shfl_xor(ssq, 32, 64);
+      rs = rsqrtf(ssq / (float)K + p.eps);
+    }
+  }
+  if constexpr (OUTP) {
+    static_for<NOB>([&](auto ob_) {
+      static_for<4>([&](auto g_) {
+        constexpr int ob = decltype(ob_)::value, gq = decltype(g_)::value;
+        areg_write4<AO + 16 * ob + 4 * gq>(__builtin_bit_cast(u32x4, xres[ob][gq]));
+      });
+    });
+  } else {
+    static_for<NOB>([&](auto ob_) { areg_zero16<AO + 16 * decltype(ob_)::value>(); });
+  }
+  warm_end();
+  asm volatile("s_waitcnt vmcnt(0) lgkmcnt(0)" ::: "memory");
+  KD_BARRIER();
+  constexpr int NWO = OUTP ? 2 * NKU : 0;
+  auto issue_wo = [&](int q, int j) {
+    const char* src = p.Wo + (size_t)q * STG + wid * (PB * 1024) + j * 1024 + lane * 16;
+    char* dst = smem + (q % NSTG) * STG + wid * (PB * 1024) + j * 1024;
+    __builtin_amdgcn_global_load_lds((const __attribute__((address_space(1))) void*)src, (__attribute__((address_space(3))) void*)dst, 16, 0, 0);
+  };
+  if constexpr (OUTP) {
+#pragma unroll
+    for (int q = 0; q < PDIST; ++q)
+#pragma unroll
+      for (int j = 0; j < PB; ++j) issue_wo(q, j);
+  } else {
+#pragma unroll
+    for (int s = EARLY; s < PDIST; ++s)
+#pragma unroll
+      for (int j = 0; j < PB; ++j) issue_rel(0, s, j);
+  }
+  if (probe) p.clk[4] = __builtin_amdgcn_s_memtime();
+
+  const int o0 = swz64(l31, lh), o1 = swz64(l31, 2 + lh);
+  f32x16 acc[4];
+  bf16x8 wh[2][4], wl[2][4];
+  auto read_frags = [&](int slot, int h, bf16x8 (&fh)[4], bf16x8 (&fl)[4]) {
+    const char* st = smem + slot * STG + (h ? o1 : o0);
+#pragma unroll
+    for (int j = 0; j < 4; ++j) {
+      fh[j] = *reinterpret_cast<const bf16x8*>(st + j * 32 * 64);
+      fl[j] = *reinterpret_cast<const bf16x8*>(st + IMG + j * 32 * 64);
+    }
+  };
+  auto next_stage_in = [&]() {
+    wait_vm(PB * (PDIST - 2));
+    KD_BARRIER();
+  };
+  wait_vm(PB * (PDIST - 1));
+  KD_BARRIER();
+  read_frags(0, 0, wh[0], wl[0]);
+  if constexpr (OUTP) {
+    constexpr std::integral_constant<int, 0> I0{};
+    constexpr std::integral_constant<int, 1> I1{};
+    constexpr std::integral_constant<int, 2> I2{};
+    constexpr std::integral_constant<int, 3> I3{};
+    static_for<NWO>([&](auto q_) {
+      constexpr int q = decltype(q_)::value, ntile = q / NKU, ks = q % NKU;
+      auto oo = [&](auto b_, auto j_, bool w_lo, auto al_) {
+        constexpr int b = decltype(b_)::value, j = decltype(j_)::value, al = decltype(al_)::value, c = 2 * ks + b;
+        mfma_acc_aa<AO + 16 * (4 * ntile + j), 8 * c + 4 * al>(w_lo ? wl[b][j] : wh[b][j]);
+      };
+      auto request = [&](int j) {
+        if constexpr (q + PDIST < NWO) issue_wo(q + PDIST, j);
+        else issue_rel(0, q + PDIST - NWO, j);
+      };
+      oo(I0, I0, true, I0);
+      __builtin_amdgcn_sched_barrier(0);
+      read_frags(q % NSTG, 1, wh[1], wl[1]);
+      __builtin_amdgcn_sched_barrier(0);
+      oo(I0, I1, true, I0); oo(I0, I2, true, I0); oo(I0, I3, true, I0);
+      oo(I0, I0, false, I1); oo(I0, I1, false, I1); oo(I0, I2, false, I1); oo(I0, I3, false, I1);
+      oo(I0, I0, false, I0); oo(I0, I1, false, I0); oo(I0, I2, false, I0); oo(I0, I3, false, I0);
+      __builtin_amdgcn_sched_barrier(0);
+      next_stage_in();
+      oo(I1, I0, true, I0);
+      __builtin_amdgcn_sched_barrier(0);
+      read_frags((q + 1) % NSTG, 0, wh[0], wl[0]);
+      __builtin_amdgcn_sched_barrier(0);
+      oo(I1, I1, true, I0); oo(I1, I2, true, I0);
+      request(0);
+      __builtin_amdgcn_sched_barrier(0);
+      oo(I1, I3, true, I0); oo(I1, I0, false, I1); oo(I1, I1, false, I1);
+      request(1);
+      __builtin_amdgcn_sched_barrier(0);
+      oo(I1, I2, false, I1); oo(I1, I3, false, I1); oo(I1, I0, false, I0);
+      request(2);
+      __builtin_amdgcn_sched_barrier(0);
+      oo(I1, I1, false, I0); oo(I1, I2, false, I0);
+      request(3);
+      oo(I1, I3, false, I0);
+      __builtin_amdgcn_sched_barrier(0);
+    });
+    asm volatile("s_nop 15\n\ts_nop 3" ::: "memory");
+    {
+      const char* scl = smem + NSTG * STG + wid * SCL;
+      const int r_first = min(pn.row(wid * 32), p.M - 1), r_last = min(pn.row(wid * 32 + 31), p.M - 1);
+      const bool uni = p.scale_stride == 0 || r_first / p.rows_per_sample == r_last / p.rows_per_sample;
+      const float* sg = uni ? nullptr : p.scale + (size_t)(rowc / p.rows_per_sample) * p.scale_stride + 4 * lh;
+      const float* sl = reinterpret_cast<const float*>(scl) + 4 * lh;
+      float ssq = 0.f;
+      static_for<NOB>([&](auto ob_) {
+        constexpr int ob = decltype(ob_)::value;
+        f32x4 v[4], sc[4];
+        static_for<4>([&](auto g_) { v[decltype(g_)::value] = areg_read4<AO + 16 * ob + 4 * decltype(g_)::value>(); });
+#pragma unroll
+        for (int g = 0; g < 4; ++g) sc[g] = uni ? *reinterpret_cast<const f32x4*>(sl + 32 * ob + 8 * g) : *reinterpret_cast<const f32x4*>(sg + 32 * ob + 8 * g);
+#pragma unroll
+        for (int g = 0; g < 4; ++g)
+#pragma unroll
+          for (int e = 0; e < 4; ++e) ssq = fmaf(v[g][e], v[g][e], ssq);
+        static_for<2>([&](auto hc_) {
+          constexpr int hc = decltype(hc_)::value;
+          u32x4 hi, lo;
+          split8(v[2 * hc] * sc[2 * hc], v[2 * hc + 1] * sc[2 * hc + 1], hi, lo);
+          areg_write4<8 * (2 * ob + hc)>(hi);
+          areg_write4<8 * (2 * ob + hc) + 4>(lo);
+        });
+      });
+      ssq += __shfl_xor(ssq, 32, 64);
+      rs = rsqrtf(ssq / (float)K + p.eps);
+    }
+  }
+  const float rsh = 0.5f * rs;
+
+  for (int t = 0; t < T; ++t) {
+    const int sbase = t * UNIT;
+    const int slot0 = sbase % NSTG;
+    if (probe && t == 2) p.clk[8] = __builtin_amdgcn_s_memtime();
+    static_for<NKU>([&](auto ks_) {
+      constexpr int ks = decltype(ks_)::value;
+      const int slot = (slot0 + ks) % NSTG, nslot = (slot0 + ks + 1) % NSTG;
+      auto mm = [&](auto b_, int j, bool w_lo, auto a_lo_) {
+        constexpr int b = decltype(b_)::value, al = decltype(a_lo_)::value, c = 2 * ks + b;
+        const bf16x8& w = w_lo ? wl[b][j] : wh[b][j];
+        constexpr bool first = ks == 0 && b == 0;
+        if constexpr (AG) {
+          if (first && w_lo) mfma_ag0<8 * c + 4 * al>(acc[j], w);
+          else mfma_ag<8 * c + 4 * al>(acc[j], w);
+        } else {
+          if (first && w_lo) mfma_vv0(acc[j], w, al ? a_lo[c] : a_hi[c]);
+          else mfma_vv(acc[j], w, al ? a_lo[c] : a_hi[c]);
+        }
+      };
+      constexpr std::integral_constant<int, 0> I0{};
+      constexpr std::integral_constant<int, 1> I1{};
+      mm(I0, 0, true, I0);
+      __builtin_amdgcn_sched_barrier(0);
+      read_frags(slot, 1, wh[1], wl[1]);
+      __builtin_amdgcn_sched_barrier(0);
+#pragma unroll
+      for (int j = 1; j < 4; ++j) mm(I0, j, true, I0);
+#pragma unroll
+      for (int j = 0; j < 4; ++j) mm(I0, j, false, I1);
+#pragma unroll
+      for (int j = 0; j < 4; ++j) mm(I0, j, false, I0);
+      __builtin_amdgcn_sched_barrier(0);
+      next_stage_in();
+      mm(I1, 0, true, I0);
+      __builtin_amdgcn_sched_barrier(0);
+      read_frags(nslot, 0, wh[0], wl[0]);
+      __builtin_amdgcn_sched_barrier(0);
+      mm(I1, 1, true, I0);
+      mm(I1, 2, true, I0);
+      issue_rel(t, ks + PDIST, 0);
+      __builtin_amdgcn_sched_barrier(0);
+      mm(I1, 3, true, I0);
+      mm(I1, 0, false, I1);
+      mm(I1, 1, false, I1);
+      issue_rel(t, ks + PDIST, 1);
+      __builtin_amdgcn_sched_barrier(0);
+      mm(I1, 2, false, I1);
+      mm(I1, 3, false, I1);
+      mm(I1, 0, false, I0);
+      issue_rel(t, ks + PDIST, 2);
+      __builtin_amdgcn_sched_barrier(0);
+      mm(I1, 1, false, I0);
+      mm(I1, 2, false, I0);
+      issue_rel(t, ks + PDIST, 3);
+      mm(I1, 3, false, I0);
+      __builtin_amdgcn_sched_barrier(0);
+    });
+    asm volatile("s_nop 15\n\ts_nop 3" : "+v"(acc[0]), "+v"(acc[1]), "+v"(acc[2]), "+v"(acc[3]));
+    if (probe && t == 0) p.clk[5] = __builtin_amdgcn_s_memtime();
+    if (probe && t == 2) p.clk[9] = __builtin_amdgcn_s_memtime();
+
+    bf16x8 hf_hi[4], hf_lo[4];
+#pragma unroll
+    for (int jj = 0; jj < 2; ++jj)
+#pragma unroll
+      for (int hc = 0; hc < 2; ++hc) {
+        f32x4 v0, v1;
+        const int r0 = 8 * hc;
+        {
+          const f32x2 a = geglu_pair(f32x2{acc[2 * jj][r0], acc[2 * jj][r0 + 1]} * rsh, f32x2{acc[2 * jj + 1][r0], acc[2 * jj + 1][r0 + 1]} * rs);
+          const f32x2 b = geglu_pair(f32x2{acc[2 * jj][r0 + 2], acc[2 * jj][r0 + 3]} * rsh, f32x2{acc[2 * jj + 1][r0 + 2], acc[2 * jj + 1][r0 + 3]} * rs);
+          v0 = f32x4{a.x, a.y, b.x, b.y};
+        }
+        {
+          const f32x2 a = geglu_pair(f32x2{acc[2 * jj][r0 + 4], acc[2 * jj][r0 + 5]} * rsh, f32x2{acc[2 * jj + 1][r0 + 4], acc[2 * jj + 1][r0 + 5]} * rs);
+          const f32x2 b = geglu_pair(f32x2{acc[2 * jj][r0 + 6], acc[2 * jj][r0 + 7]} * rsh, f32x2{acc[2 * jj + 1][r0 + 6], acc[2 * jj + 1][r0 + 7]} * rs);
+          v1 = f32x4{a.x, a.y, b.x, b.y};
+        }
+        u32x4 hi, lo;
+        split8(v0, v1, hi, lo);
+        hf_hi[2 * jj + hc] = __builtin_bit_cast(bf16x8, hi);
+        hf_lo[2 * jj + hc] = __builtin_bit_cast(bf16x8, lo);
+      }
+    asm volatile("s_nop 7" : "+v"(hf_hi[0]), "+v"(hf_hi[1]), "+v"(hf_hi[2]), "+v"(hf_hi[3]), "+v"(hf_lo[0]), "+v"(hf_lo[1]), "+v"(hf_lo[2]), "+v"(hf_lo[3]));
+    __builtin_amdgcn_sched_barrier(0);
+    if (probe && t == 2) p.clk[10] = __builtin_amdgcn_s_memtime();
+
+    static_for<NKD>([&](auto v_) {
+      constexpr int v = decltype(v_)::value, ntile = v >> 1, kk = v & 1;
+      const int slot = (slot0 + NKU + v) % NSTG, nslot = (slot0 + NKU + v + 1) % NSTG;
+      auto dd = [&](auto b_, auto j_, bool w_lo, bool h_lo) {
+        constexpr int b = decltype(b_)::value, j = decltype(j_)::value;
+        const bf16x8& w = w_lo ? wl[b][j] : wh[b][j];
+        const bf16x8& h = h_lo ? hf_lo[2 * kk + b] : hf_hi[2 * kk + b];
+        mfma_acc_ag<AO + 16 * (4 * ntile + j)>(w, h);
+      };
+      constexpr std::integral_constant<int, 0> I0{};
+      constexpr std::integral_constant<int, 1> I1{};
+      constexpr std::integral_constant<int, 2> I2{};
+      constexpr std::integral_constant<int, 3> I3{};
+      dd(I0, I0, true, false);
+      __builtin_amdgcn_sched_barrier(0);
+      read_frags(slot, 1, wh[1], wl[1]);
+      __builtin_amdgcn_sched_barrier(0);
+      dd(I0, I1, true, false); dd(I0, I2, true, false); dd(I0, I3, true, false);
+      dd(I0, I0, false, true); dd(I0, I1, false, true); dd(I0, I2, false, true); dd(I0, I3, false, true);
+      dd(I0, I0, false, false); dd(I0, I1, false, false); dd(I0, I2, false, false); dd(I0, I3, false, false);
+      __builtin_amdgcn_sched_barrier(0);
+      next_stage_in();
+      dd(I1, I0, true, false);
+      __builtin_amdgcn_sched_barrier(0);
+      read_frags(nslot, 0, wh[0], wl[0]);
+      __builtin_amdgcn_sched_barrier(0);
+      dd(I1, I1, true, false); dd(I1, I2, true, false);
+      issue_rel(t, NKU + v + PDIST, 0);
+      __builtin_amdgcn_sched_barrier(0);
+      dd(I1, I3, true, false); dd(I1, I0, false, true); dd(I1, I1, false, true);
+      issue_rel(t, NKU + v + PDIST, 1);
+      __builtin_amdgcn_sched_barrier(0);
+      dd(I1, I2, false, true); dd(I1, I3, false, true); dd(I1, I0, false, false);
+      issue_rel(t, NKU + v + PDIST, 2);
+      __builtin_amdgcn_sched_barrier(0);
+      dd(I1, I1, false, false); dd(I1, I2, false, false);
+      issue_rel(t, NKU + v + PDIST, 3);
+      dd(I1, I3, false, false);
+      __builtin_amdgcn_sched_barrier(0);
+    });
+    if (probe && t == 0) p.clk[6] = __builtin_amdgcn_s_memtime();
+    if (probe && t == 2) p.clk[11] = __builtin_amdgcn_s_memtime();
+  }
+  if (probe) p.clk[12] = __builtin_amdgcn_s_memtime();
+  char* strip = smem + NSTG * STG + 4 * SCL + wid * 2048;
+  float* st_row[2];
+  const float* sk_row[2];
+  bool st_ok[2];
+#pragma unroll
+  for (int it = 0; it < 2; ++it) {
+    const int r = pn.row(wid * 32 + 16 * it + (lane >> 2));
+    st_ok[it] = r < p.M;
+    st_row[it] = p.Y + (size_t)min(r, p.M - 1) * K + 4 * (lane & 3);
+    sk_row[it] = p.X + (size_t)min(r, p.M - 1) * K + 4 * (lane & 3);
+  }
+  f32x4 skip_all[NOB][2][2];
+#pragma unroll
+  for (int ob = 0; ob < NOB; ++ob)
+#pragma unroll
+    for (int hb = 0; hb < 2; ++hb)
+#pragma unroll
+      for (int it = 0; it < 2; ++it)
+        skip_all[ob][hb][it] = OUTP ? f32x4{0.f, 0.f, 0.f, 0.f} : *reinterpret_cast<const f32x4*>(sk_row[it] + 32 * ob + 16 * hb);
+  __builtin_amdgcn_sched_barrier(0);
+  asm volatile("s_waitcnt vmcnt(0)\n\ts_nop 15\n\ts_nop 3" ::: "memory");
+  static_for<NOB>([&](auto ob_) {
+    constexpr int ob = decltype(ob_)::value;
+    f32x4 blk[4];
+    static_for<4>([&](auto g_) { blk[decltype(g_)::value] = areg_read4<AO + 16 * ob + 4 * decltype(g_)::value>(); });
+#pragma unroll
+    for (int hb = 0; hb < 2; ++hb) {
+      const f32x4 (&skip)[2] = skip_all[ob][hb];
+#pragma unroll
+      for (int gg = 0; gg < 2; ++gg)
+        *reinterpret_cast<f32x4*>(strip + l31 * 64 + (((2 * gg + lh) ^ ((l31 >> 2) & 1)) << 4)) = blk[2 * hb + gg];
+#pragma unroll
+      for (int it = 0; it < 2; ++it) {
+        const int r16 = 16 * it + (lane >> 2), c = lane & 3;
+        const f32x4 o = *reinterpret_cast<const f32x4*>(strip + r16 * 64 + ((c ^ ((r16 >> 2) & 1)) << 4));
+        if (st_ok[it]) st16(st_row[it] + 32 * ob + 16 * hb, f32x4(o + skip[it]));
+      }
+    }
+  });
+  if (probe) { p.clk[2] = __builtin_amdgcn_s_memtime(); p.clk[3] = __builtin_amdgcn_s_memrealtime(); p.clk[7] = (unsigned long long)total; }
+}
+
+}
+}
```

Result: no change. 240.0, median of 6 (+1.0%).
